# NVIDIA/cuopt

Hardware: AMD Instinct MI355X
Metric: pdlp_iterations_per_sec (higher is better)
Workload: dtype f64; 1 GPU; c3: synthetic random sparse LP S(m=1000000,n=1000000,k=10,seed=2), nnz=10000000, longest row 10, CSR fp64/int32, Stable2 preset, tolerances 0 (fixed iteration budget); rows=1000000, cols=1000000, nnz=10000000, parallelism=single GPU

## Files before the change

### cuopt_amd/capi.py

```python
import ctypes as C
import os

import numpy as np

_HERE = os.path.dirname(os.path.abspath(__file__))
LIB_PATH = os.environ.get("CUOPT_AMD_LIB") or os.path.join(_HERE, "lib", "libcuopt.so")

if not os.path.exists(LIB_PATH):
    raise ImportError(
        "cuopt_amd: %s is missing -- build it with `make -C cuopt_amd/csrc` (or "
        "`python -c 'import __graft_entry__ as g; g.build()'`). There is no CPU fallback." % LIB_PATH)

lib = C.CDLL(LIB_PATH, mode=C.RTLD_GLOBAL)

CUOPT_SUCCESS, CUOPT_INVALID_ARGUMENT, CUOPT_MPS_FILE_ERROR, CUOPT_MPS_PARSE_ERROR = 0, 1, 2, 3
CUOPT_VALIDATION_ERROR, CUOPT_OUT_OF_MEMORY, CUOPT_RUNTIME_ERROR = 4, 5, 6
CUOPT_MINIMIZE, CUOPT_MAXIMIZE = 1, -1
STATUS = {0: "NoTermination", 1: "Optimal", 2: "PrimalInfeasible", 3: "DualInfeasible",
          4: "IterationLimit", 5: "TimeLimit", 6: "NumericalError", 7: "PrimalFeasible",
          8: "FeasibleFound", 9: "ConcurrentLimit"}

c_int, c_double, c_void_p, c_char_p = C.c_int32, C.c_double, C.c_void_p, C.c_char_p
P = C.POINTER


def _f64(a):
    return np.ascontiguousarray(a, dtype=np.float64)


def _i32(a):
    return np.ascontiguousarray(a, dtype=np.int32)


def _ptr(a):
    return None if a is None else a.ctypes.data_as(c_void_p)


class Ctl(C.Structure):
    _fields_ = [("step_size", c_double), ("primal_weight", c_double), ("tau", c_double),
                ("sigma", c_double), ("sum_weights", c_double), ("last_interaction", c_double),
                ("last_movement", c_double), ("last_dx2", c_double), ("last_dy2", c_double),
                ("k", c_int), ("cur", c_int), ("pending_avg", c_int), ("steps_taken", c_int),
                ("attempts", c_int), ("target_steps", c_int), ("error", c_int),
                ("its_since_restart", c_int)]


class StepParams(C.Structure):
    _fields_ = [("reduction_exponent", c_double), ("growth_exponent", c_double),
                ("primal_distance_smoothing", c_double), ("dual_distance_smoothing", c_double)]


class LP(C.Structure):
    _fields_ = [("m", c_int), ("n", c_int), ("offsets", c_void_p), ("indices", c_void_p),
                ("values", c_void_p), ("c", c_void_p), ("lo", c_void_p), ("hi", c_void_p),
                ("lb", c_void_p), ("ub", c_void_p), ("maximize", c_int),
                ("objective_offset", c_double)]


class Hyper(C.Structure):
    _fields_ = [("initial_step_size_scaling", c_double), ("ruiz_iterations", c_int),
                ("do_pock_chambolle", c_int), ("do_ruiz", c_int), ("alpha_pock_chambolle", c_double),
                ("artificial_restart_threshold", c_double),
                ("compute_initial_step_size_before_scaling", c_int),
                ("compute_initial_primal_weight_before_scaling", c_int),
                ("initial_primal_weight_c_scaling", c_double),
                ("initial_primal_weight_b_scaling", c_double), ("major_iteration", c_int),
                ("min_iteration_restart", c_int), ("restart_strategy", c_int),
                ("never_restart_to_average", c_int), ("reduction_exponent", c_double),
                ("growth_exponent", c_double), ("primal_weight_update_smoothing", c_double),
                ("sufficient_reduction_for_restart", c_double),
                ("necessary_reduction_for_restart", c_double), ("primal_importance", c_double),
                ("primal_distance_smoothing", c_double), ("dual_distance_smoothing", c_double),
                ("compute_last_restart_before_new_primal_weight", c_int),
                ("artificial_restart_in_main_loop", c_int), ("rescale_for_restart", c_int),
                ("update_primal_weight_on_initial_solution", c_int),
                ("update_step_size_on_initial_solution", c_int),
                ("handle_some_primal_gradients_on_finite_bounds_as_residuals", c_int),
                ("project_initial_primal", c_int),
                ("algorithm", c_int), ("halpern_power_max_products", c_int),
                ("halpern_step_safety", c_double), ("halpern_power_tolerance", c_double)]


class Halpern(C.Structure):
    _fields_ = [("r", c_double), ("r_first", c_double), ("r2", c_double), ("r2_min", c_double),
                ("k", c_int), ("reserved", c_int)]


class SolverSettings(C.Structure):
    _fields_ = [("absolute_gap_tolerance", c_double), ("relative_gap_tolerance", c_double),
                ("absolute_primal_tolerance", c_double), ("relative_primal_tolerance", c_double),
                ("absolute_dual_tolerance", c_double), ("relative_dual_tolerance", c_double),
                ("iteration_limit", c_int), ("time_limit", c_double),
                ("per_constraint_residual", c_int), ("first_primal_feasible", c_int),
                ("initial_step_size", c_double), ("initial_primal_weight", c_double),
                ("initial_k", c_int), ("use_graph", c_int), ("detect_infeasibility", c_int),
                ("strict_infeasibility", c_int), ("primal_infeasible_tolerance", c_double),
                ("dual_infeasible_tolerance", c_double), ("save_best_primal_so_far", c_int),
                ("log_to_console", c_int), ("log_file", c_char_p), ("unbounded_from_feasible_iterates", c_int),
                ("accept_enabled", c_int), ("accept_tolerance", c_double * 6),
                ("relative_primal_tolerance_factor", c_double), ("relative_dual_tolerance_factor", c_double),
                ("batch_lanes", c_int), ("halpern_resident", c_int), ("halpern_batch", c_int), ("halpern_lockstep", c_int)]


class SolverSettingsWithRays(SolverSettings):
    _fields_ = [("halpern_infeasibility", c_int)]


assert SolverSettingsWithRays.halpern_infeasibility.offset == SolverSettings.halpern_lockstep.offset + C.sizeof(c_int)


class Result(C.Structure):
    _fields_ = [("status", c_int), ("steps_taken", c_int), ("attempted_steps", c_int),
                ("returned_average", c_int), ("num_restarts", c_int), ("num_major_iterations", c_int),
                ("primal_objective", c_double), ("dual_objective", c_double), ("gap", c_double),
                ("relative_gap", c_double), ("l2_primal_residual", c_double),
                ("l2_dual_residual", c_double), ("l2_relative_primal_residual", c_double),
                ("l2_relative_dual_residual", c_double), ("max_primal_ray_infeasibility", c_double),
                ("max_dual_ray_infeasibility", c_double), ("primal_ray_linear_objective", c_double),
                ("dual_ray_linear_objective", c_double), ("initial_step_size", c_double),
                ("initial_primal_weight", c_double), ("step_size", c_double),
                ("primal_weight", c_double), ("norm_b", c_double), ("norm_c", c_double),
                ("setup_seconds", c_double), ("loop_seconds", c_double),
                ("accepted_at_looser_tolerances", c_int), ("gpus", c_int)]

    def as_dict(self):
        d = {k: getattr(self, k) for k, _ in self._fields_}
        d["status_name"] = STATUS.get(self.status, str(self.status))
# ... 141 lines not shown
if hasattr(lib, "pdlpdev_debug_attempts"):
    _proto("pdlpdev_debug_attempts", c_int, c_void_p, c_int, P(Ctl))
_proto("pdlpdev_clear_error", c_int, c_void_p)
_proto("pdlpdev_set_graph_mode", c_int, c_void_p, c_int)
_proto("pdlpdev_prepare_graphs", c_int, c_void_p)
_proto("pdlpdev_flush_average", c_int, c_void_p)
_proto("pdlpdev_make_average", c_int, c_void_p, c_int)
_proto("pdlpdev_eval", c_int, c_void_p, c_int, c_int, c_double, c_double, c_void_p)
_proto("pdlpdev_restart", c_int, c_void_p, c_int, c_int, c_void_p)
_proto("pdlpdev_major_eval", c_int, c_void_p, c_int, c_int, c_double, c_double, c_void_p, c_void_p)
if hasattr(lib, "pdlpdev_loop_stats"):
    _proto("pdlpdev_loop_stats", c_int, c_void_p, c_void_p)
    _proto("pdlpdev_run_period", c_int, c_void_p, c_int, c_void_p, c_void_p, c_void_p, c_void_p, c_void_p)
_proto("pdlpdev_save_best", c_int, c_void_p, c_int)
_proto("pdlpdev_trust_region_bounds", c_int, c_void_p, c_int, c_double, c_double, c_double, c_double, c_double, c_double, c_int, c_void_p)
_proto("pdlpdev_eval_infeasibility", c_int, c_void_p, c_int, c_int, c_void_p)
_proto("pdlpdev_get_solution", c_int, c_void_p, c_int, c_void_p, c_void_p, c_void_p)
_proto("pdlpdev_download", C.c_int64, c_void_p, c_int, c_void_p, C.c_int64)
_proto("pdlpdev_upload", C.c_int64, c_void_p, c_int, c_void_p, C.c_int64)
_proto("pdlpdev_spmv", c_int, c_void_p, c_int, c_void_p, c_void_p)
_proto("pdlpdev_time_kernel", c_int, c_void_p, c_int, c_int, P(c_double))
_proto("pdlpdev_synchronize", c_int, c_void_p)
_proto("pdlpdev_device_bytes", C.c_int64, c_void_p)
_proto("cuoptamd_dual_simplex", c_int, c_void_p, c_double, c_int, c_void_p, c_void_p, c_void_p, c_void_p, c_void_p, c_void_p, c_void_p)
_proto("cuoptamd_dual_simplex_from", c_int, c_void_p, c_void_p, c_void_p, c_double, c_int, c_void_p, c_void_p, c_void_p, c_void_p, c_void_p, c_void_p, c_void_p)
_proto("pdlpdev_shard_dataflow", c_int, c_void_p)
_proto("pdlpdev_shard_transport", c_int, c_void_p)
_proto("pdlpdev_shard_wire_bytes", c_int, c_void_p, c_void_p)
_proto("pdlpdev_dense_info", c_int, c_void_p, c_void_p)
_proto("pdlpdev_layout_info", c_int, c_void_p, c_void_p)
_proto("pdlpdev_comm_abort", c_int, c_void_p)
if hasattr(lib, "pdlpdev_shard_slice"):
    _proto("pdlpdev_shard_slice", c_int, c_void_p, P(c_int), P(c_int))
    _proto("pdlpdev_owner_layout_info", c_int, c_void_p, c_void_p)
_proto("pdlpdev_analyze", c_int, P(c_void_p), c_int, c_int, c_int, c_void_p, c_void_p, c_void_p, c_int)
_proto("pdlpdev_analysis_info", c_int, c_void_p, c_void_p)
_proto("pdlpdev_analysis_maps", c_int, c_void_p, c_void_p, c_void_p)
_proto("pdlpdev_analysis_download", c_int, c_void_p, c_int, c_void_p, c_void_p, c_void_p)
_proto("pdlpdev_create_from_analysis", c_int, P(c_void_p), c_void_p, c_void_p, c_void_p, c_void_p, c_void_p, c_void_p)
_proto("pdlpdev_analysis_destroy", None, c_void_p)
_proto("pdlpdev_debug_sort_pairs", c_int, c_int, C.c_int64, c_void_p, c_void_p, c_int, c_void_p, c_void_p)
_proto("pdlpdev_debug_scan", c_int, c_int, C.c_int64, c_void_p, c_void_p)
_proto("pdlpdev_debug_layout_checksums", c_int, c_void_p, c_void_p)
_proto("cuoptamd_solver_clone", c_int, c_void_p, c_void_p, c_void_p, c_void_p, c_void_p, c_void_p, P(c_void_p))
_proto("cuoptamd_batch_create", c_int, c_void_p, c_int, P(c_void_p))
_proto("cuoptamd_batch_advance", c_int, c_void_p, c_int, c_void_p)
_proto("cuoptamd_batch_destroy", None, c_void_p)
_proto("cuoptamd_batch_reset", c_int, c_void_p, c_void_p, c_void_p, c_void_p, c_void_p)
_proto("cuoptamd_batch_get_solutions", c_int, c_void_p, c_void_p, c_void_p, c_void_p)
_proto("cuoptamd_batch_branch", c_int, c_void_p, c_void_p, c_void_p, c_void_p)
_proto("cuoptamd_batch_solution_views", c_int, c_void_p, c_void_p, c_void_p, c_void_p)
_proto("cuoptamd_batch_device", c_void_p, c_void_p)
_proto("cuoptamd_batch_stats", c_int, c_void_p, c_void_p)
_proto("cuoptamd_batch_solve_last_path", C.c_char_p)
_proto("pdlpdev_small_batch_create", c_int, P(c_void_p), P(c_void_p), c_int)
_proto("pdlpdev_small_batch_destroy", None, c_void_p)
_proto("pdlpdev_create_share_stream", None, c_void_p)
_proto("pdlpdev_debug_ipc_export", c_int, c_int, c_int, c_void_p, P(c_void_p))
_proto("pdlpdev_debug_ipc_store", c_int, c_int, c_void_p, c_int, c_double)
_proto("pdlpdev_debug_ipc_wait", c_int, c_int, c_void_p, c_int, c_double)
_proto("pdlpdev_resident_size", c_int, c_int, c_int, C.c_int64)
if hasattr(lib, "pdlpdev_resident_tier"):
    _proto("pdlpdev_resident_tier", c_int, c_int, c_int, C.c_int64)
_proto("pdlpdev_batch_time_kernels", c_int, c_void_p, c_int, c_void_p)
_proto("pdlpdev_synthetic_lp", c_int, c_int, c_int, c_int, c_int, C.c_uint64, *([c_void_p] * 8))

if hasattr(lib, "pdlpdev_set_halpern"):
    _proto("pdlpdev_create_no_resident", None, c_int)
    _proto("pdlpdev_set_halpern", c_int, c_void_p, c_int)
    _proto("pdlpdev_spectral_norm", c_int, c_void_p, c_double, c_int, P(c_double), P(c_int))
    _proto("pdlpdev_halpern_restart", c_int, c_void_p, c_double, c_void_p, P(Ctl))
    _proto("pdlpdev_get_halpern", c_int, c_void_p, P(Halpern))
if hasattr(lib, "cuoptamd_solver_get_ray"):
    _proto("cuoptamd_solver_get_ray", c_int, c_void_p, c_void_p, c_void_p)
    _proto("pdlpdev_set_halpern_rays", c_int, c_void_p, c_int)
    _proto("pdlpdev_halpern_eval_infeasibility", c_int, c_void_p, c_int, c_void_p)
    _proto("pdlpdev_halpern_get_ray", c_int, c_void_p, c_void_p, c_void_p)
PDLP_SOLVER_MODE_HALPERN1 = 4

BUF = {n: i for i, n in enumerate(
    ["X", "Y", "X_OTHER", "Y_OTHER", "ATY", "ATY_OTHER", "XBAR", "SUM_X", "SUM_Y", "AVG_X", "AVG_Y",
     "DROW", "DCOL", "A_VALUES", "AT_VALUES", "C", "LB", "UB", "LO", "HI", "RC_CURRENT", "RC_AVERAGE",
     "LAST_RESTART_X", "LAST_RESTART_Y", "ATY_U_CURRENT", "ATY_U_AVERAGE", "LAST_RESTART_ATY",
     "AX_U_CURRENT", "AX_U_AVERAGE"])}
KERNEL = {n: i for i, n in enumerate(
    ["PRIMAL", "SPMV_A_DUAL", "SPMV_AT_STEP", "STEP_DECISION", "SPMV_A_PLAIN", "SPMV_AT_PLAIN"])}
EV = {n: i for i, n in enumerate(
    ["CX", "DUAL_SUM", "PRES2", "DRES2", "X2", "Y2", "LINF_PRES_REL", "LINF_DRES_REL"])}
CURRENT, AVERAGE = 0, 1
LAST_RESTART = 2


class CuOptError(RuntimeError):
    def __init__(self, code, msg=""):
        super().__init__("cuopt error %d %s" % (code, msg))
        self.code = code


def device_count():
    return int(lib.pdlpdev_device_count())


def device_info(dev=0):
    name = C.create_string_buffer(256)
    cus, mem = c_int(), C.c_int64()
    rc = lib.pdlpdev_device_info(dev, name, 256, C.byref(cus), C.byref(mem))
    if rc != 0:
        raise CuOptError(rc, lib.pdlpdev_last_error().decode())
    return dict(name=name.value.decode(), compute_units=cus.value, hbm_bytes=mem.value)


class Problem:

    def __init__(self, handle):
        self.handle = handle

    @classmethod
    def read(cls, path):
        h = c_void_p()
        rc = lib.cuOptReadProblem(os.fsencode(path), C.byref(h))
        if rc != CUOPT_SUCCESS:
            raise CuOptError(rc, "cuOptReadProblem(%s)" % path)
        return cls(h)

    @classmethod
    def from_dict(cls, p, ranged=True):
        m, n = int(p["m"]), int(p["n"])
        keep = [_i32(p["offsets"]), _i32(p["indices"]), _f64(p["values"]), _f64(p["c"]),
                _f64(p["lb"]), _f64(p["ub"])]
        vt = p.get("var_types")
        vt = (b"C" * n) if vt is None else bytes(bytearray(np.asarray(vt, dtype=np.uint8)))
        h = c_void_p()
        sense = CUOPT_MAXIMIZE if p.get("maximize", False) else CUOPT_MINIMIZE
        off = float(p.get("objective_offset", 0.0))
        if ranged:
            lo, hi = _f64(p["lo"]), _f64(p["hi"])
            rc = lib.cuOptCreateRangedProblem(m, n, sense, off, _ptr(keep[3]), _ptr(keep[0]),
                                              _ptr(keep[1]), _ptr(keep[2]), _ptr(lo), _ptr(hi),
                                              _ptr(keep[4]), _ptr(keep[5]), vt, C.byref(h))
        else:
            rt = bytes(bytearray(np.asarray(p["row_types"], dtype=np.uint8)))
            rhs = _f64(p["rhs"])
            rc = lib.cuOptCreateProblem(m, n, sense, off, _ptr(keep[3]), _ptr(keep[0]), _ptr(keep[1]),
                                        _ptr(keep[2]), rt, _ptr(rhs), _ptr(keep[4]), _ptr(keep[5]), vt,
                                        C.byref(h))
        if rc != CUOPT_SUCCESS:
            raise CuOptError(rc, "cuOptCreate*Problem")
        return cls(h)

    def _int(self, fn):
        v = c_int()
        rc = fn(self.handle, C.byref(v))
        if rc != 0:
            raise CuOptError(rc)
        return v.value

    @property
    def m(self):
        return self._int(lib.cuOptGetNumConstraints)

    @property
    def n(self):
        return self._int(lib.cuOptGetNumVariables)

    @property
    def nnz(self):
        return self._int(lib.cuOptGetNumNonZeros)
# ... 779 lines not shown
```

### cuopt_amd/csrc/kernels_batch.hip

```cpp
#include <cstring>
#include <hip/hip_runtime.h>

#include "batch_common.hpp"
#include "pdlp_ctx.hpp"

#define LAUNCH_CHECK() HIP_TRY(hipGetLastError())

__global__ void k_step_decision_batch(const pdlpdev_decision_args* __restrict__ args);
__global__ void k_set_target(pdlpdev_ctl* ctl, int target);
__global__ void k_set_error(pdlpdev_ctl* ctl);

namespace {

template <int K>
__global__ void __launch_bounds__(kBT) kb_primal(const BatchLp* __restrict__ lp, int n, double* __restrict__ xK)
{
  __shared__ double tile[kBT][K + 1];
  using WL = WaveLps<K>;
  const int wave = threadIdx.x >> 6, lane = threadIdx.x & 63, sub = WL::sub(wave);
  for (int t0 = blockIdx.x * kBT; t0 < n; t0 += gridDim.x * kBT) {
#pragma unroll
    for (int pass = 0; pass < WL::PASSES; ++pass) {
      const int l       = WL::lp(wave, pass);
      const BatchLp L   = lp[l];
// ... 423 lines not shown
    return batch_halpern_enqueue_tail(K, s, ps, pt, b->lp_dev, b->hl_dev, b->xK, b->yK);
  }
  if (ev) {
    JagView ajv = A.jv, tjv = T.jv;
    int aP = A.P, tP = T.P;
    void* a0[] = {&b->lp_dev, &n, &b->xK};
    void* a1[] = {&aw, &arow0, &c0->A.hot.off, &c0->A.hot.idx, &c0->A.hot.val, &b->lp_dev, &b->xK, &b->yK};
    void* a2[] = {&tw, &trow0, &c0->At.hot.off, &c0->At.hot.idx, &c0->At.hot.val, &b->lp_dev, &b->yK};
    void* j1[] = {&ajv, &aP, &b->lp_dev, &b->xK, &b->yK};
    void* j2[] = {&tjv, &tP, &b->lp_dev, &b->yK};
    void* a3[] = {&b->dargs_dev};
    HIP_TRY(hipExtLaunchKernel((const void*)kb_primal<K>, dim3(pgrid), dim3(kBT), a0, 0, s, ev[0], ev[1], 0));
    if (A.jag)
      HIP_TRY(hipExtLaunchKernel(batch_jag_kernel<K>(A, true), jgrid(A), dim3(A.jv.waves * 64), j1, A.lds, s, ev[2], ev[3], 0));
    else
      HIP_TRY(hipExtLaunchKernel(ap ? (const void*)kb_a_dual<K, 8> : (const void*)kb_a_dual<K, 4>, dim3(aw), dim3(kBT), a1, 0, s, ev[2], ev[3], 0));
    if (T.jag)
      HIP_TRY(hipExtLaunchKernel(batch_jag_kernel<K>(T, false), jgrid(T), dim3(T.jv.waves * 64), j2, T.lds, s, ev[4], ev[5], 0));
    else
      HIP_TRY(hipExtLaunchKernel(tp ? (const void*)kb_at_step<K, 8> : (const void*)kb_at_step<K, 4>, dim3(tw), dim3(kBT), a2, 0, s, ev[4], ev[5], 0));
    HIP_TRY(hipExtLaunchKernel((const void*)k_step_decision_batch, dim3(K), dim3(1024), a3, 0, s, ev[6], ev[7], 0));
    return 0;
  }
  kb_primal<K><<<pgrid, kBT, 0, s>>>(b->lp_dev, n, b->xK);
  if (A.jag && A.jv.waves == 16) kbj_a_dual<K, 16><<<jgrid(A), 1024, A.lds, s>>>(A.jv, A.P, b->lp_dev, b->xK, b->yK);
  else if (A.jag) kbj_a_dual<K, 8><<<jgrid(A), 512, A.lds, s>>>(A.jv, A.P, b->lp_dev, b->xK, b->yK);
  else if (ap) kb_a_dual<K, 8><<<aw, kBT, 0, s>>>(aw, arow0, c0->A.hot.off, c0->A.hot.idx, c0->A.hot.val, b->lp_dev, b->xK, b->yK);
  else kb_a_dual<K, 4><<<aw, kBT, 0, s>>>(aw, arow0, c0->A.hot.off, c0->A.hot.idx, c0->A.hot.val, b->lp_dev, b->xK, b->yK);
  if (T.jag && T.jv.waves == 16) kbj_at_step<K, 16><<<jgrid(T), 1024, T.lds, s>>>(T.jv, T.P, b->lp_dev, b->yK);
  else if (T.jag) kbj_at_step<K, 8><<<jgrid(T), 512, T.lds, s>>>(T.jv, T.P, b->lp_dev, b->yK);
  else if (tp) kb_at_step<K, 8><<<tw, kBT, 0, s>>>(tw, trow0, c0->At.hot.off, c0->At.hot.idx, c0->At.hot.val, b->lp_dev, b->yK);
  else kb_at_step<K, 4><<<tw, kBT, 0, s>>>(tw, trow0, c0->At.hot.off, c0->At.hot.idx, c0->At.hot.val, b->lp_dev, b->yK);
  k_step_decision_batch<<<K, 1024, 0, s>>>(b->dargs_dev);
  LAUNCH_CHECK();
  return 0;
}

static int batch_enqueue(pdlpdev_batch* b, hipEvent_t* ev = nullptr)
{
  return b->K == 16  ? batch_enqueue_attempt<16>(b, ev)
         : b->K == 8 ? batch_enqueue_attempt<8>(b, ev)
         : b->K == 4 ? batch_enqueue_attempt<4>(b, ev)
                     : batch_enqueue_attempt<2>(b, ev);
}

static int batch_graph(pdlpdev_batch* b, int attempts, hipGraphExec_t* out)
{
  auto it = b->graphs.find(attempts);
  if (it != b->graphs.end()) {
    *out = it->second;
    return 0;
  }
  hipGraph_t graph;
  HIP_TRY(hipStreamBeginCapture(b->stream, hipStreamCaptureModeThreadLocal));
  int rc = 0;
  for (int i = 0; i < attempts && rc == 0; ++i) rc = batch_enqueue(b);
  hipError_t e = hipStreamEndCapture(b->stream, &graph);
  if (rc != 0) return rc;
  HIP_TRY(e);
  hipGraphExec_t exec;
  HIP_TRY(hipGraphInstantiate(&exec, graph, nullptr, nullptr, 0));
  HIP_TRY(hipGraphDestroy(graph));
  b->graphs[attempts] = exec;
  *out                = exec;
  return 0;
}

extern "C" {

int pdlpdev_clone_shared(pdlpdev_ctx** out, pdlpdev_ctx* parent)
{
  if (!out || !parent) return fail(-1, "pdlpdev_clone_shared: null argument");
  if (!parent->scaled) return fail(-1, "pdlpdev_clone_shared: the parent has not been scaled yet");
  if (parent->comm || parent->small_resident || parent->dense.on) return fail(-7, "pdlpdev_clone_shared: not for sharded, resident or dense-segment contexts");
  HIP_TRY(hipSetDevice(parent->device));
  HIP_TRY(hipStreamSynchronize(parent->stream));
  pdlpdev_ctx* c = new pdlpdev_ctx(*parent);
  *out           = c;
  c->allocs.clear(), c->graphs.clear(), c->scratch.clear();
  c->shared_with_parent = true;
  c->parent = nullptr;
  c->scal_h = nullptr, c->ctl_h = nullptr;
  c->halpern = false, c->lraty = nullptr, c->hal = nullptr, c->hal_h = nullptr;
  c->clones_alive = 0, c->batches_alive = 0, c->rows_private = false;
  c->bytes = 0, c->slab = nullptr, c->slab_cap = c->slab_used = 0, c->arena = nullptr, c->arena_used = 0, c->first_chunk = nullptr;
  c->bestx = c->besty = c->bestrc = nullptr;
  c->prof_armed = false, c->prof_used = 0, c->rejected_in_a_row = 0;
  for (hipEvent_t& e : c->prof_ev) e = nullptr;
  HIP_TRY(hipHostMalloc((void**)&c->scal_h, kScalars * sizeof(double) + sizeof(pdlpdev_ctl)));
  c->ctl_h = (pdlpdev_ctl*)(c->scal_h + kScalars);
  HIP_TRY(hipMalloc((void**)&c->arena, kArenaChunk));
  HIP_TRY(hipMemsetAsync(c->arena, 0, kArenaChunk, c->stream));
  c->first_chunk = c->arena;
  const int m = c->m, n = c->n;
  {
    const size_t bytes = (24 * ((size_t)n + kSlicePad + 32) + 15 * ((size_t)m + 32)) * sizeof(double);
    if ((int64_t)m + n >= 262144 && hipMalloc((void**)&c->slab, bytes) == hipSuccess) {
      c->allocs.push_back(c->slab);
      c->slab_cap = bytes;
      HIP_TRY(hipMemsetAsync(c->slab, 0, bytes, c->stream));
    } else {
      c->slab = nullptr;
      (void)hipGetLastError();
    }
  }
  auto own_copy = [&](double** p, size_t count) -> int {
    const double* src = *p;
    TRY(dev_alloc(c, p, count));
    HIP_TRY(hipMemcpyAsync(*p, src, count * sizeof(double), hipMemcpyDeviceToDevice, c->stream));
    return 0;
  };
  TRY(own_copy(&c->lb, n)); TRY(own_copy(&c->lb_u, n)); TRY(own_copy(&c->ub, n)); TRY(own_copy(&c->ub_u, n));
  c->rows_aliased = true, c->parent = parent, c->clones_alive = 0;
  parent->clones_alive += 1;
  parent->rows_private = false;
  for (int i = 0; i < 2; ++i) {
    TRY(dev_alloc(c, &c->x[i], (size_t)n + kSlicePad)); TRY(dev_alloc(c, &c->y[i], m));
    TRY(dev_alloc(c, &c->aty[i], (size_t)n + kSlicePad)); TRY(dev_alloc(c, &c->rc[i], n));
  }
  TRY(dev_alloc(c, &c->xbar, (size_t)n + kSlicePad)); TRY(dev_alloc(c, &c->sumx, (size_t)n + kSlicePad)); TRY(dev_alloc(c, &c->sumy, m));
  TRY(dev_alloc(c, &c->avgx, n)); TRY(dev_alloc(c, &c->avgy, m));
  TRY(dev_alloc(c, &c->lrx, n)); TRY(dev_alloc(c, &c->lry, m));
  TRY(dev_alloc(c, &c->tmp_n, n)); TRY(dev_alloc(c, &c->tmp_m, m));
  for (int i = 0; i < 3; ++i) {
    TRY(dev_alloc(c, &c->ax_u[i], m));
    TRY(dev_alloc(c, &c->aty_u[i], n));
  }
  TRY(dev_alloc(c, &c->rc_scratch, n));
  TRY(dev_alloc(c, &c->A.part, (size_t)8 * c->A.max_partials()));
  TRY(dev_alloc(c, &c->At.part, (size_t)8 * c->At.max_partials()));
  TRY(dev_alloc(c, &c->part_g, (size_t)8 * 2048));
  TRY(dev_alloc(c, &c->scal, kScalars));
  TRY(dev_alloc(c, &c->ctl, 1));
  TRY(dev_alloc(c, &c->ar_buf, (size_t)n + kSlicePad));
  HIP_TRY(hipMemcpyAsync(c->ctl, parent->ctl, sizeof(pdlpdev_ctl), hipMemcpyDeviceToDevice, c->stream));
  HIP_TRY(hipStreamSynchronize(c->stream));
  return 0;
}

int pdlpdev_batch_create(pdlpdev_batch** out, pdlpdev_ctx** ctx, int K)
{
  if (!out || !ctx || (K != 2 && K != 4 && K != 8 && K != 16)) return fail(-1, "pdlpdev_batch_create: K must be 2, 4, 8 or 16");
  pdlpdev_ctx* c0 = ctx[0];
  for (int l = 0; l < K; ++l)
    for (int q = 0; q < l; ++q)
      if (ctx[q] == ctx[l]) return fail(-1, "pdlpdev_batch_create: LP %d and LP %d are the same context (two lanes would share one set of iterates)", q, l);
  for (int l = 0; l < K; ++l) {
    pdlpdev_ctx* c = ctx[l];
    if (!c || c->A.hot.off != c0->A.hot.off || c->At.hot.off != c0->At.hot.off || c->A.pan.v.row0 != c0->A.pan.v.row0 || c->A.jag.v.row0 != c0->A.jag.v.row0 ||
        c->At.jag.v.row0 != c0->At.jag.v.row0 || c->A.jag.v.val != c0->A.jag.v.val || c->At.jag.v.val != c0->At.jag.v.val || c->stream != c0->stream)
      return fail(-1, "pdlpdev_batch_create: the contexts do not share one matrix (pdlpdev_clone_shared)");
  }
  int nhalpern = 0;
  for (int l = 0; l < K; ++l) nhalpern += ctx[l]->halpern ? 1 : 0;
  if (nhalpern != 0 && nhalpern != K)
    return fail(-7, "pdlpdev_batch_create: not eligible (the batch mixes %d contexts in reflected Halpern mode with %d in the averaging iteration: a lockstep "
                    "attempt runs one of the two)", nhalpern, K - nhalpern);
  const bool halpern = nhalpern == K;
  for (int l = 0; halpern && l < K; ++l)
    if (!ctx[l]->hal || !ctx[l]->hal_h || !ctx[l]->lraty) return fail(-1, "pdlpdev_batch_create: LP %d is in reflected Halpern mode without its anchor (pdlpdev_set_halpern)", l);
  if ((int64_t)std::max(c0->m, c0->n) * K >= ((int64_t)1 << 32))
    return fail(-7, "pdlpdev_batch_create: not eligible (the interleaved vectors are addressed with 32-bit element offsets: max(m, n) * K < 2^32)");
  pdlpdev_batch::Side side[2];
  HIP_TRY(hipSetDevice(c0->device));
  const pdlpdev_ctx::MatrixSide* const matrix[2] = {&c0->A, &c0->At};
  for (int t = 0; t < 2; ++t) {
// ... 232 lines not shown
```

### cuopt_amd/csrc/kernels_panel.hip

```cpp
#include <hip/hip_runtime.h>

#include "pdlp_kernel_decls.hpp"
#include "pdlp_layouts.hpp"
#include "pdlp_setup.hpp"
#include "spmv_panel.hpp"

template <bool SEG>
__global__ void __launch_bounds__(kPanelThreads)
k_panel_a_dual(PanelView P, const pdlpdev_ctl* __restrict__ ctl, const double* __restrict__ xbar,
               double* __restrict__ y0, double* __restrict__ y1, const double* __restrict__ lo,
               const double* __restrict__ hi, double* __restrict__ sumy, double* __restrict__ part, double* __restrict__ ycopy,
               const p2pdev::Push* __restrict__ push)
{
  if (!loop_active(ctl)) return;
  DualEpilogue e = DualEpilogue::make(ctl, y0, y1, lo, hi, sumy, ycopy, push);
  panel_block<SEG>(P, xbar, e, part);
  if (push) p2pdev::count_exchange(push);
}

template <bool SEG>
__global__ void __launch_bounds__(kPanelThreads)
k_panel_at_step(PanelView P, const pdlpdev_ctl* __restrict__ ctl, const double* __restrict__ y0,
                const double* __restrict__ y1, const double* __restrict__ x0,
                const double* __restrict__ x1, double* __restrict__ aty0, double* __restrict__ aty1,
                double* __restrict__ part)
{
  if (!loop_active(ctl)) return;
  StepEpilogue e = StepEpilogue::make(ctl, x0, x1, aty0, aty1);
  panel_block<SEG>(P, ctl->cur ? y0 : y1 , e, part);
}

template <bool SEG>
__global__ void __launch_bounds__(kPanelThreads)
k_panel_a_halpern(PanelView P, const pdlpdev_ctl* __restrict__ ctl, const double* __restrict__ xbar,
                  double* __restrict__ y0, double* __restrict__ y1, const double* __restrict__ lo,
                  const double* __restrict__ hi, HalpernArgs h, double* __restrict__ part)
{
  if (!loop_active(ctl)) return;
  HalpernDualEpilogue e = HalpernDualEpilogue::make(ctl, y0, y1, lo, hi, h);
  panel_block<SEG>(P, xbar, e, part);
}

template <bool SEG>
__global__ void __launch_bounds__(kPanelThreads)
k_panel_at_halpern(PanelView P, const pdlpdev_ctl* __restrict__ ctl, double* __restrict__ x0, double* __restrict__ x1,
                   double* __restrict__ aty0, double* __restrict__ aty1, HalpernArgs h, double* __restrict__ part)
{
  if (!loop_active(ctl)) return;
  HalpernStepEpilogue e = HalpernStepEpilogue::make(ctl, x0, x1, aty0, aty1, h);
  panel_block<SEG>(P, h.ty , e, part);
}

template <bool SEG>
__global__ void __launch_bounds__(kPanelThreads)
k_panel_at_cur(PanelView P, const pdlpdev_ctl* __restrict__ ctl, const double* __restrict__ y0,
               const double* __restrict__ y1, double* __restrict__ aty0, double* __restrict__ aty1,
               double* __restrict__ out_override, int use_next)
{
  const int cur = ctl->cur ^ (use_next ? 1 : 0);
  StoreEpilogue e = StoreEpilogue::iterate(cur, aty0, aty1, out_override);
  panel_block<SEG>(P, cur ? y1 : y0, e, nullptr);
}

template <bool SEG>
__global__ void __launch_bounds__(kPanelThreads)
k_panel_plain(PanelView P, const double* __restrict__ vec, double* __restrict__ out)
{
  StoreEpilogue e{out};
  panel_block<SEG>(P, vec, e, nullptr);
}

template <bool SEG>
__global__ void __launch_bounds__(kPanelThreads)
k_panel_eval_primal(PanelView P, const pdlpdev_ctl* __restrict__ ctl, int which,
                    const double* __restrict__ x0, const double* __restrict__ x1,
                    const double* __restrict__ avgx, const double* __restrict__ y0,
                    const double* __restrict__ y1, const double* __restrict__ avgy,
                    const double* __restrict__ dr, const double* __restrict__ lo_u,
                    const double* __restrict__ hi_u, double eps_rel, double* __restrict__ linf_rows,
                    double* __restrict__ ax_out, double* __restrict__ part)
{
  if (period_guard_skips(ctl, which)) return;
  const int cur = ctl->cur;
  const double* xv = evaluated(cur, which, x0, x1, avgx);
  const double* yv = evaluated(cur, which, y0, y1, avgy);
  EvalPrimalEpilogue e{yv, dr, lo_u, hi_u, eps_rel, linf_rows, ax_out};
  panel_block<SEG>(P, xv, e, part);
}

template <bool SEG>
__global__ void __launch_bounds__(kPanelThreads)
k_panel_eval_dual(PanelView P, const pdlpdev_ctl* __restrict__ ctl, int which,
                  const double* __restrict__ x0, const double* __restrict__ x1,
                  const double* __restrict__ avgx, const double* __restrict__ y0,
                  const double* __restrict__ y1, const double* __restrict__ avgy, EvalDualCore core,
                  double* __restrict__ part)
{
  if (period_guard_skips(ctl, which)) return;
  const int cur = ctl->cur;
// ... 331 lines not shown
```

### cuopt_amd/csrc/pdlp_create.hip

```cpp
#include "pdlp_ctx.hpp"
#include "pdlp_layouts.hpp"
#include "pdlp_setup.hpp"

__global__ void k_fill(int64_t n, double* __restrict__ d, double v);
int sync_panel_values(pdlpdev_ctx* c);
int resident_tier(int m, int n, int64_t nnz);

static thread_local int g_create_sharded = 0;
static thread_local int g_create_no_resident = 0;
static thread_local int g_create_batch_lanes = 0;

static int create_impl(pdlpdev_ctx** out, int device, int32_t m, int32_t n, const int32_t* a_offsets,
                       const int32_t* a_indices, const double* a_values, const int32_t* at_offsets,
                       const int32_t* at_indices, const double* at_values,
                       void (*transpose_ready)(void*), void* user, const double* c, const double* lo,
                       const double* hi, const double* lb, const double* ub, pdlpdev_analysis* an);

extern "C" {

const char* pdlpdev_last_error(void) { return g_err.c_str(); }
void pdlpdev_create_hint(int sharded) { g_create_sharded = sharded; }
void pdlpdev_create_no_resident(int no_resident) { g_create_no_resident = no_resident; }
void pdlpdev_create_batch_lanes(int lanes) { g_create_batch_lanes = lanes; }
static thread_local pdlpdev_ctx* g_create_stream_donor = nullptr;
// ... 446 lines not shown
      if (!hT_off.empty()) T.off = hT_off.data(), T.idx = hT_idx.data();
      rbt = build_row_blocks(n, T.off);
      wlap("row blocks");
      if (walk) at_rc = layout_walk(ctx, P, T);
    };
    struct Join {
      std::thread t;
      ~Join() { if (t.joinable()) t.join(); }
    } worker;
    if (at_thread) worker.t = std::thread(at_side, true);
    {
      LayoutSide A;
      init_side(A, &ctx->A, 0);
      A.off = A_off, A.idx = A_idx, A.d_off = ctx->A.hot.off, A.d_idx = ctx->A.hot.idx, A.d_val = ctx->A.hot.val, A.lap = lap;
      A.first_seg = DH.on ? &DH.first_seg : nullptr;
      TRY(layout_walk(ctx, P, A));
      TRY(upload_side(ctx, P, A));
      if (ctx->A.pan.on && DH.on) TRY(own_segments(ctx, DH, A.ph));
      lap("upload layouts A");
    }
    if (at_thread) worker.t.join();
    else at_side(false);
    lap("wait for the A^T side");
    if ((int64_t)at_offsets[n] != ctx->nnz) return fail(-1, "pdlpdev_create: A and A^T disagree on nnz");
    if (!an) {
      TRY(upload_i32(ctx, &ctx->At.full.off, at_offsets, (size_t)n + 1));
      TRY(upload_i32(ctx, &ctx->At.full.idx, at_indices, nnz, 8));
      TRY(upload_f64(ctx, &ctx->At.full.val, at_values, nnz, 8));
    }
    ctx->At.nlong = (int)lat.size();
    if (ctx->At.nlong) TRY(upload_i32(ctx, &ctx->At.longs, lat.data(), lat.size()));
    const bool hot_t = !hT_off.empty();
    ctx->At.hot = ctx->At.full;
    ctx->At.hot_nnz = (int64_t)T.off[n];
    if (hot_t) {
      TRY(upload_i32(ctx, &ctx->At.hot.off, T.off, (size_t)n + 1));
      TRY(upload_i32(ctx, &ctx->At.hot.idx, T.idx, (size_t)ctx->At.hot_nnz, 8));
      TRY(dev_alloc(ctx, &ctx->At.hot.val, (size_t)ctx->At.hot_nnz + 8));
      TRY(upload_i32(ctx, &ctx->dense.s_perm_at, hT_perm.data(), hT_perm.size()));
    }
    if (DH.on) TRY(dev_alloc(ctx, &ctx->At.dense_add, (size_t)n));
    ctx->At.nb = (int)rbt.size() / 2 - 1;
    TRY(upload_i32(ctx, &ctx->At.rb, rbt.data(), rbt.size()));
    lap("upload A^T");
    T.d_off = ctx->At.hot.off, T.d_idx = ctx->At.hot.idx, T.d_val = ctx->At.hot.val;
    TRY(at_thread ? at_rc : layout_walk(ctx, P, T));
    TRY(upload_side(ctx, P, T));
    if (ctx->At.pan.on && DH.on) TRY(column_segments(ctx, DH, T.ph));
    lap("upload layouts A^T");
    HIP_TRY(hipStreamSynchronize(ctx->stream));
  }
  {
    const char* small_env = getenv("CUOPT_AMD_SMALL");
    const int tier        = resident_tier(m, n, ctx->nnz);
    ctx->eval_reuse_aty   = cuopt_amd::tune_int("eval_reuse_aty", 1) != 0;
    ctx->small_resident   = tier >= 0 && !(small_env && atoi(small_env) == 0) && !ctx->A.dense_add && !ctx->At.dense_add && !g_create_no_resident;
    g_create_no_resident  = 0;
    if (small_env && atoi(small_env) != 0 && tier < 0)
      return fail(-1, "CUOPT_AMD_SMALL=1: the LP does not fit the resident kernel (m, n <= 2048, nnz <= 4096 ...)");
  }
  ctx->slab_cap += slab_rest;
  for (pdlpdev_ctx::MatrixSide* s : {&ctx->A, &ctx->At}) {
    s->pan.v.dense_add = s->jag.v.dense_add = s->pb.v.dense_add = s->dense_add;
    if (s->pan.v.dn_own_seg || s->pan.v.dn_pan_ptr) s->pan.v.dense_add = nullptr;
    TRY(dev_alloc(ctx, &s->part, (size_t)8 * s->max_partials()));
  }
  TRY(dev_alloc(ctx, &ctx->part_g, (size_t)8 * 2048));
  TRY(dev_alloc(ctx, &ctx->scal, kScalars));
  TRY(dev_alloc(ctx, &ctx->ctl, 1));
  TRY(dev_alloc(ctx, &ctx->ar_buf, (size_t)n + kSlicePad));
  lap("partial buffers");
  k_fill<<<grid_for(m), kBlock, 0, ctx->stream>>>(m, ctx->dr, 1.0);
  k_fill<<<grid_for(n), kBlock, 0, ctx->stream>>>(n, ctx->dc, 1.0);
  HIP_TRY(hipGetLastError());
  lap("fill D");
  TRY(sync_panel_values(ctx));
  lap("panel values (permute)");
  if (P.mode == LayoutPolicy::kTimed) {
    TRY(pick_layout(ctx, &ctx->A, ctx->tmp_n, ctx->tmp_m));
    lap("layout autotune A");
    TRY(pick_layout(ctx, &ctx->At, ctx->tmp_m, ctx->tmp_n));
    lap("layout autotune");
  }
  HIP_TRY(hipStreamSynchronize(ctx->stream));
  scratch_free(ctx);
  return 0;
}

extern "C" {

void pdlpdev_destroy(pdlpdev_ctx* ctx)
{
  if (!ctx) return;
  (void)hipSetDevice(ctx->device);
  if (ctx->stream) (void)hipStreamSynchronize(ctx->stream);
  scratch_free(ctx);
  for (auto& kv : ctx->graphs) (void)hipGraphExecDestroy(kv.second);
  if (ctx->shared_with_parent && ctx->parent) ctx->parent->clones_alive -= 1;
  if (ctx->batches_alive > 0)
    fprintf(stderr, "[cuopt_amd] pdlpdev_destroy: %d batch(es) still hold this context -- destroy the batch before its members\n", ctx->batches_alive);
  if (ctx->clones_alive > 0)
    fprintf(stderr, "[cuopt_amd] pdlpdev_destroy: %d clone(s) of this context are still alive -- they alias its matrices and must be destroyed first\n", ctx->clones_alive);
  for (void* mapped : ctx->p2p.opened) (void)hipIpcCloseMemHandle(mapped);
  if (ctx->p2p.base) (void)hipFree(ctx->p2p.base);
  if (ctx->comm && !ctx->soft) comm_cache::release(ctx->comm_key);
  for (void* p : ctx->allocs) (void)hipFree(p);
  if (ctx->hal_h) (void)hipHostFree(ctx->hal_h);
  const bool whole = ctx->stream && ctx->scal_h && ctx->first_chunk && !ctx->shared_with_parent && !ctx->stream_borrowed;
  if (!(whole && give_recycled(Recycled{ctx->device, ctx->stream, ctx->scal_h, ctx->first_chunk}))) {
    if (ctx->first_chunk) (void)hipFree(ctx->first_chunk);
    if (ctx->scal_h) (void)hipHostFree(ctx->scal_h);
    if (ctx->stream && !ctx->shared_with_parent && !ctx->stream_borrowed) (void)hipStreamDestroy(ctx->stream);
  }
  delete ctx;
}

}
```

### cuopt_amd/csrc/pdlp_ctx.hpp

```cpp
#pragma once
#include <hip/hip_runtime.h>
#include <hip/hip_ext.h>

#include <tuple>
#include <utility>

#include <dlfcn.h>
#include <unistd.h>
#include <mutex>
#include <math.h>
#include <stdarg.h>
#include <stdio.h>
#include <string.h>

#include <algorithm>
#include <chrono>
#include <map>
#include <memory>
#include <string>
#include <vector>

#include "host_parallel.hpp"
#include "pdlp_kernels.hpp"
#include "pdlp_epilogues.hpp"
// ... 276 lines not shown
    int32_t* rb = nullptr;
    int nb = 0;
    int32_t* longs = nullptr;
    int nlong = 0;
    Panels pan;
    Jag jag;
    Pb pb;
    double* part = nullptr;
    double* dense_add = nullptr;
    enum Layout { kStream = 0, kPanel = 1, kJag = 3, kPb = 4 };
    Layout layout() const { return pb.on ? kPb : jag.on ? kJag : pan.on ? kPanel : kStream; }
    int partials() const
    {
      switch (layout()) {
        case kPb: return pb.v.B;
        case kJag: return jag.v.nblk + jag.v.nlong;
        case kPanel: return pan.v.W;
        default: return nb;
      }
    }
    int max_partials() const { return std::max({nb, pb.on ? pb.v.B : 0, pan.on ? pan.v.W : 0, jag.on ? jag.v.nblk + jag.v.nlong : 0, 1}); }
    void info(int32_t out[3]) const
    {
      out[0] = layout();
      switch (layout()) {
        case kPb: out[1] = pb.v.B, out[2] = (int)(100.0 * (pb.pad - 1.0) + 0.5); break;
        case kJag: out[1] = jag.v.nblk, out[2] = (int)(100.0 * jag.saving + 0.5); break;
        case kPanel: out[1] = pan.v.W, out[2] = pan.v.S; break;
        default: out[1] = nb, out[2] = 1;
      }
    }
    bool fuses_dense() const { return pan.on && (pan.v.dn_own_seg != nullptr || pan.v.dn_pan_ptr != nullptr); }
  };
  MatrixSide A, At;
  struct Dense {
    bool on = false;
    int nrows = 0, nseg = 0, ntiles = 0;
    int64_t nent = 0;
    int32_t *row = nullptr, *row_seg = nullptr;
    int32_t *seg_row = nullptr, *seg_c0 = nullptr, *seg_len = nullptr, *seg_ptr = nullptr;
    int32_t *ch_seg = nullptr, *ch_k0 = nullptr, *row_ch = nullptr;
    double* ch_part = nullptr;
    int nchunks = 0;
    int32_t *tile_ptr = nullptr, *tile_seg = nullptr, *tile_id = nullptr;
    int32_t *perm = nullptr, *s_perm_a = nullptr, *s_perm_at = nullptr;
    double* val = nullptr;
    int32_t* tile_slot = nullptr;
  } dense;
  double *c = nullptr, *lb = nullptr, *ub = nullptr, *lo = nullptr, *hi = nullptr;
  struct UniformBounds {
    int lb_same = 0, ub_same = 0;
    double lb = 0.0, ub = 0.0;
  } ubd;
  void note_uniform_bounds(const double* lb_host, const double* ub_host)
  {
    auto same = [&](const double* v, int* flag, double* value) {
      if (!v) return;
      *flag = 0;
      if (n <= 0) return;
      const double v0 = v[0];
      if (!(v0 == 0.0 || std::isinf(v0))) return;
      constexpr int kParts = 16;
      bool differs[kParts] = {false};
      cuopt_amd::parallel_tasks(kParts, [&](int t) {
        const int32_t a = (int32_t)((int64_t)n * t / kParts), b = (int32_t)((int64_t)n * (t + 1) / kParts);
        for (int32_t j = a; j < b; ++j)
          if (v[j] != v0) {
            differs[t] = true;
            return;
          }
      }, (int64_t)n * 4);
      for (bool d : differs)
        if (d) return;
      *flag = 1, *value = v0;
    };
    same(lb_host, &ubd.lb_same, &ubd.lb);
    same(ub_host, &ubd.ub_same, &ubd.ub);
  }
  double *c_u = nullptr, *lb_u = nullptr, *ub_u = nullptr, *lo_u = nullptr, *hi_u = nullptr;
  double *dr = nullptr, *dc = nullptr;
  bool scaled = false;
  double *x[2] = {nullptr, nullptr}, *y[2] = {nullptr, nullptr}, *aty[2] = {nullptr, nullptr};
  double *xbar = nullptr, *sumx = nullptr, *sumy = nullptr, *avgx = nullptr, *avgy = nullptr;
  double *lrx = nullptr, *lry = nullptr, *rc[2] = {nullptr, nullptr};
  double *tmp_n = nullptr, *tmp_m = nullptr;
  double *ax_u[3] = {nullptr, nullptr, nullptr}, *aty_u[3] = {nullptr, nullptr, nullptr};
  double* rc_scratch = nullptr;
  double *bestx = nullptr, *besty = nullptr, *bestrc = nullptr;
  double *part_g = nullptr;
  double *scal = nullptr;
  double *scal_h = nullptr;
  pdlpdev_ctl *ctl = nullptr, *ctl_h = nullptr;
  pdlpdev_step_params sp = {0.3, 0.6, 0.5, 0.5};
  bool halpern = false;
  double* lraty = nullptr;
  pdlpdev_halpern *hal = nullptr, *hal_h = nullptr;
  bool halpern_rays = false;
  rccl::comm_t comm = nullptr;
  softcomm::Comm* soft = nullptr;
  std::string comm_key;
  int rank = 0, world = 1;
  double* ar_buf = nullptr;
  bool rsag = false;
  int slice = 0;
  double* rs_buf = nullptr;
  double* rs_scal = nullptr;
  bool owner = false;
  int ypad = 0;
  double* ygather = nullptr;
  MatrixSide Oc;
  struct Halo {
    bool on = false;
    std::vector<int32_t> recv_off[2], recv_cnt[2], send_off[2], send_cnt[2];
    int64_t bytes = 0, bytes_allgather = 0;
  } halo;
  struct P2P {
    bool on = false;
    char* base = nullptr;
    size_t bytes = 0;
    size_t off_x = 0, off_y = 0, off_s = 0, off_f = 0;
    p2pdev::Peers peers{};
    std::vector<void*> opened;
    unsigned long long* epoch = nullptr;
    int* fault = nullptr;
    p2pdev::Push* push_dev = nullptr;
    p2pdev::Push push_host[p2pdev::kKinds];
  } p2p;
  bool prof_armed = false;
  static constexpr int kProfPairs = 8;
  hipEvent_t prof_ev[2 * kProfPairs] = {};
  int prof_used = 0;
  int rejected_in_a_row = 0;
  bool aty_valid = false, ctl_h_current = false;
  int eval_reuse_aty = 1;
  int spare_attempts = 0;
  int64_t stat_eval_reused = 0, stat_eval_product = 0, stat_loop_syncs = 0, stat_empty_attempts = 0;
  int use_graph = 1;
  int batch_lanes = 0;
  bool comm_warm = false;
  bool graph_comm_failed = false;
  char* slab = nullptr;
  size_t slab_cap = 0, slab_used = 0;
  char* arena = nullptr;
  char* first_chunk = nullptr;
  bool stream_borrowed = false;
  size_t arena_used = 0;
  bool small_resident = false;
  bool shared_with_parent = false;
  pdlpdev_ctx* parent = nullptr;
  bool rows_aliased = false;
  int clones_alive = 0;
  bool rows_private = false;
  int batches_alive = 0;
  std::map<int, hipGraphExec_t> graphs;
  std::vector<void*> allocs;
  int64_t bytes = 0;
  struct Scratch {
    void* p;
    size_t bytes;
    bool busy;
  };
  std::vector<Scratch> scratch;
};
inline int scratch_take(pdlpdev_ctx* c, void** p, size_t bytes)
{
  bytes = std::max<size_t>(bytes, 256);
// ... 137 lines not shown
```

### cuopt_amd/csrc/pdlp_device.hip

```cpp
#include "pdlp_ctx.hpp"
#include "pdlp_layouts.hpp"
#include "pdlp_setup.hpp"
#include "halpern_decision.hpp"


__global__ void __launch_bounds__(kBlock) k_fill(int64_t n, double* __restrict__ d, double v)
{
  for (int64_t i = blockIdx.x * (int64_t)kBlock + threadIdx.x; i < n; i += (int64_t)gridDim.x * kBlock)
    d[i] = v;
}
__global__ void __launch_bounds__(kBlock) k_scale_vectors(int n, int m, double* __restrict__ c,
                                                          double* __restrict__ lb,
                                                          double* __restrict__ ub,
                                                          const double* __restrict__ dc,
                                                          double* __restrict__ lo,
                                                          double* __restrict__ hi,
                                                          const double* __restrict__ dr)
{
  const int tot = n > m ? n : m;
  for (int i = blockIdx.x * kBlock + threadIdx.x; i < tot; i += gridDim.x * kBlock) {
    if (i < n) {
      c[i]  = c[i] * dc[i];
      lb[i] = lb[i] / dc[i];
      ub[i] = ub[i] / dc[i];
// ... 1 lines not shown
    if (i < m) {
      lo[i] = lo[i] * dr[i];
      hi[i] = hi[i] * dr[i];
    }
  }
}
__global__ void __launch_bounds__(kBlock) k_scale_bounds(int n, int m, double* lb, double* ub,
                                                         const double* __restrict__ dc, double* lo, double* hi,
                                                         const double* __restrict__ dr)
{
  const int tot = n > m ? n : m;
  for (int i = blockIdx.x * kBlock + threadIdx.x; i < tot; i += gridDim.x * kBlock) {
    if (i < n) {
      if (lb) lb[i] = lb[i] / dc[i];
      if (ub) ub[i] = ub[i] / dc[i];
    }
    if (i < m) {
      if (lo) lo[i] = lo[i] * dr[i];
      if (hi) hi[i] = hi[i] * dr[i];
    }
  }
}
__global__ void __launch_bounds__(kBlock) k_div_inplace(int n, double* __restrict__ v,
                                                        const double* __restrict__ d)
{
  for (int i = blockIdx.x * kBlock + threadIdx.x; i < n; i += gridDim.x * kBlock) v[i] = v[i] / d[i];
}
__global__ void __launch_bounds__(kBlock) k_div_to(int n, double* __restrict__ out, const double* __restrict__ v,
                                                   const double* __restrict__ d)
{
  for (int i = blockIdx.x * kBlock + threadIdx.x; i < n; i += gridDim.x * kBlock) out[i] = v[i] / d[i];
}
__global__ void __launch_bounds__(kBlock) k_clamp(int n, double* __restrict__ x,
                                                  const double* __restrict__ lb,
                                                  const double* __restrict__ ub)
{
  for (int i = blockIdx.x * kBlock + threadIdx.x; i < n; i += gridDim.x * kBlock)
    x[i] = dmin(dmax(x[i], lb[i]), ub[i]);
}

template <int MODE>
__global__ void __launch_bounds__(kBlock) k_reduce(int64_t n, const double* __restrict__ a,
                                                   const double* __restrict__ b,
                                                   double* __restrict__ part)
{
  __shared__ double red[8];
  double acc[1] = {0.0};
  for (int64_t i = blockIdx.x * (int64_t)kBlock + threadIdx.x; i < n; i += (int64_t)gridDim.x * kBlock) {
    if (MODE == 0) {
      const double v = fabs(a[i]);
      acc[0] = v > acc[0] ? v : acc[0];
    } else if (MODE == 1) {
      acc[0] += a[i] * a[i];
    } else if (MODE == 2) {
      const double v = combine_bounds(a[i], b[i]);
      acc[0] += v * v;
    } else {
      const double v = a[i] - b[i];
      acc[0] += v * v;
    }
  }
  if (MODE == 0)
    block_reduce<MaxOp, 1>(acc, red);
  else
    block_reduce<SumOp, 1>(acc, red);
  if (threadIdx.x == 0) part[blockIdx.x] = acc[0];
}
__global__ void __launch_bounds__(kBlock) k_dot(int64_t n, const double* __restrict__ a, const double* __restrict__ b,
                                                double* __restrict__ part)
{
  __shared__ double red[8];
  double acc[1] = {0.0};
  for (int64_t i = blockIdx.x * (int64_t)kBlock + threadIdx.x; i < n; i += (int64_t)gridDim.x * kBlock) acc[0] += a[i] * b[i];
  block_reduce<SumOp, 1>(acc, red);
  if (threadIdx.x == 0) part[blockIdx.x] = acc[0];
}
__global__ void __launch_bounds__(kBlock) k_finalize(const double* __restrict__ part, int nb, int nq,
                                                     unsigned op_mask, double* __restrict__ out)
{
  __shared__ double red[8];
  finalize_rows(part, nb, nq, op_mask, out, red);
}

__global__ void __launch_bounds__(kBlock)
k_primal(int n, const pdlpdev_ctl* __restrict__ ctl, double* __restrict__ x0, double* __restrict__ x1,
         const double* __restrict__ aty0, const double* __restrict__ aty1,
         const double* __restrict__ c, const double* __restrict__ lb, const double* __restrict__ ub,
         double* __restrict__ xbar, double* __restrict__ sumx, const p2pdev::Push* __restrict__ push, pdlpdev_ctx::UniformBounds ubd)
{
  if (!loop_active(ctl)) return;
  const int cur       = ctl->cur;
  const double tau    = ctl->tau;
  const double weight = ctl->step_size;
  const bool pend     = ctl->pending_avg != 0;
  const double* __restrict__ x   = cur ? x1 : x0;
  double* __restrict__ xn        = cur ? x0 : x1;
  const double* __restrict__ aty = cur ? aty1 : aty0;
  for (int j = blockIdx.x * kBlock + threadIdx.x; j < n; j += gridDim.x * kBlock) {
    const double xj       = x[j];
    const double gradient = c[j] - aty[j];
    double next           = xj - (tau * gradient);
    next                  = dmax(dmin(next, ubd.ub_same ? ubd.ub : ub[j]), ubd.lb_same ? ubd.lb : lb[j]);
    xn[j]                 = next;
    const double xb       = next - xj + next;
    xbar[j]               = xb;
    if (push)
      for (int q = 0; q < push->world; ++q)
        if (push->wants(q, j)) p2pdev::put(push->slot(q) + j, xb);
    if (pend) sumx[j] = sumx[j] + weight * xj;
  }
  if (push) p2pdev::count_exchange(push);
}



__global__ void __launch_bounds__(kBlock)
k_step_stats(int n, int nbg, const pdlpdev_ctl* __restrict__ ctl, const double* __restrict__ reduced,
             const double* __restrict__ x0, const double* __restrict__ x1, double* __restrict__ aty0,
             double* __restrict__ aty1, double* __restrict__ part)
{
  __shared__ double red[12];
  if (!loop_active(ctl)) return;
  const int cur = ctl->cur;
  const double* __restrict__ x   = cur ? x1 : x0;
  const double* __restrict__ xn  = cur ? x0 : x1;
  const double* __restrict__ aty = cur ? aty1 : aty0;
  double* __restrict__ atyn      = cur ? aty0 : aty1;
  double acc[2] = {0.0, 0.0};
  for (int j = blockIdx.x * kBlock + threadIdx.x; j < n; j += gridDim.x * kBlock) {
    const double v  = reduced[j];
    atyn[j]         = v;
    const double dx = xn[j] - x[j];
    const double t  = v - aty[j];
    acc[0] += t * dx;
    acc[1] += dx * dx;
  }
  block_reduce<SumOp, 2>(acc, red);
  if (threadIdx.x == 0) {
    part[blockIdx.x]       = acc[0];
    part[nbg + blockIdx.x] = acc[1];
  }
}

constexpr int kDecisionThreads = 1024;
static_assert(kDecisionThreads == kHalpernDecisionThreads, "k_halpern_decision runs halpern_decision_workgroup");
__device__ __forceinline__ void step_decision_workgroup(pdlpdev_ctl* __restrict__ ctl, const double* __restrict__ part_dy, int nb_dy,
                                                        const double* __restrict__ part_t, int nb_t, const double* __restrict__ dy2_reduced,
                                                        const pdlpdev_step_params& sp)
{
  __shared__ double red[3 * 16];
  __shared__ double pw[2];
  pdlpdev_ctl lc = *ctl;
  if (!(lc.error == 0 && lc.steps_taken < lc.target_steps)) return;
  const int t = threadIdx.x;
  if (t >= kDecisionThreads - 2) {
    const double knext = (double)(lc.k + 1) + 1.0;
    pw[t - (kDecisionThreads - 2)] = pow(knext, t == kDecisionThreads - 2 ? -sp.reduction_exponent : -sp.growth_exponent);
  }
  double acc[3] = {0.0, 0.0, 0.0};
  if (dy2_reduced == nullptr) {
#pragma unroll 4
    for (int i = t; i < nb_dy; i += kDecisionThreads) acc[0] += part_dy[i];
  }
#pragma unroll 4
  for (int i = t; i < nb_t; i += kDecisionThreads) {
    acc[1] += part_t[i];
    acc[2] += part_t[nb_t + i];
  }
  block_sum_fast<3, kDecisionThreads / 64>(acc, red);
  if (t != 0) return;
  apply_step_decision(&lc, dy2_reduced ? dy2_reduced[0] : acc[0], acc[1], acc[2], sp, pw);
  *ctl = lc;
}
__global__ void __launch_bounds__(kDecisionThreads)
k_step_decision(pdlpdev_ctl* __restrict__ ctl, const double* __restrict__ part_dy, int nb_dy,
                const double* __restrict__ part_t, int nb_t, const double* __restrict__ dy2_reduced,
                pdlpdev_step_params sp)
{
  step_decision_workgroup(ctl, part_dy, nb_dy, part_t, nb_t, dy2_reduced, sp);
}
__global__ void __launch_bounds__(kDecisionThreads)
k_step_decision_batch(const pdlpdev_decision_args* __restrict__ args)
{
  const pdlpdev_decision_args a = args[blockIdx.x];
  step_decision_workgroup(a.ctl, a.part_dy, a.nb_dy, a.part_t, a.nb_t, nullptr, a.sp);
}

__global__ void __launch_bounds__(kDecisionThreads)
k_halpern_decision(pdlpdev_ctl* __restrict__ ctl, pdlpdev_halpern* __restrict__ hal, const double* __restrict__ part_dy, int nb_dy,
                   const double* __restrict__ part_t, int nb_t)
{
  halpern_decision_workgroup(ctl, hal, part_dy, nb_dy, part_t, nb_t);
}
__global__ void k_halpern_clear(pdlpdev_halpern* hal)
{
  hal->r = hal->r_first = hal->r2 = 0.0;
  hal->r2_min = __builtin_huge_val();
  hal->k = 0, hal->reserved = 0;
}
__global__ void k_halpern_restart_ctl(pdlpdev_ctl* ctl, pdlpdev_halpern* hal, double* dist2, double theta)
{
  const double dx = sqrt(dist2[0]), dy = sqrt(dist2[1]);
  dist2[0] = dx, dist2[1] = dy;
  if (theta >= 0.0 && dx > 1.0e-10 && dy > 1.0e-10) {
    const double w     = exp(theta * log(dy / dx) + (1.0 - theta) * log(ctl->primal_weight));
    ctl->primal_weight = w;
    ctl->tau           = ctl->step_size / w;
    ctl->sigma         = ctl->step_size * w;
  }
  ctl->its_since_restart = 0;
  hal->k                 = 0;
}
__global__ void __launch_bounds__(kBlock)
k_copy_current(int n, const pdlpdev_ctl* __restrict__ ctl, const double* __restrict__ v0, const double* __restrict__ v1, double* __restrict__ out)
{
  const double* __restrict__ v = ctl->cur ? v1 : v0;
  for (int i = blockIdx.x * kBlock + threadIdx.x; i < n; i += gridDim.x * kBlock) out[i] = v[i];
}
__global__ void __launch_bounds__(kBlock) k_div_by_scalar(int n, double* __restrict__ out, const double* __restrict__ v, double d)
{
  for (int i = blockIdx.x * kBlock + threadIdx.x; i < n; i += gridDim.x * kBlock) out[i] = v[i] / d;
}

__global__ void __launch_bounds__(kBlock)
k_step_decision_p2p(pdlpdev_ctl* __restrict__ ctl, const double* __restrict__ part_dy, int nb_dy, const double* __restrict__ part_t, int nb_t,
                    const double* __restrict__ landed, const unsigned long long* __restrict__ flags, int world,
                    const unsigned long long* __restrict__ epoch, int* __restrict__ fault, pdlpdev_step_params sp, const p2pdev::Push* __restrict__ push)
{
  if (!loop_active(ctl)) return;
  {
    __shared__ double red[3 * 8];
    double acc[3] = {0.0, 0.0, 0.0};
    for (int i = threadIdx.x; i < nb_dy; i += kBlock) acc[0] += part_dy[i];
    for (int i = threadIdx.x; i < nb_t; i += kBlock) {
      acc[1] += part_t[i];
      acc[2] += part_t[nb_t + i];
    }
    block_reduce<SumOp, 3>(acc, red);
    if (threadIdx.x == 0) {
      for (int q = 0; q < push->world; ++q) {
        double* d = push->slot(q);
        p2pdev::put(d, acc[0]), p2pdev::put(d + 1, acc[1]), p2pdev::put(d + 2, acc[2]);
      }
      asm volatile("s_waitcnt vmcnt(0)" ::: "memory");
      push->epoch[push->kind] = push->epoch[push->kind] + 1;
      p2pdev::raise(push);
    }
    __syncthreads();
  }
  if (!p2pdev::wait_flags(flags, world, 2, epoch)) {
    if (threadIdx.x == 0) *fault = 1, ctl->error = 1;
    return;
  }
  if (threadIdx.x != 0) return;
  double sum[3] = {0.0, 0.0, 0.0};
  for (int q = 0; q < world; ++q)
    for (int k = 0; k < 3; ++k) sum[k] += __hip_atomic_load(landed + 4 * q + k, __ATOMIC_RELAXED, __HIP_MEMORY_SCOPE_SYSTEM);
  pdlpdev_ctl lc = *ctl;
  apply_step_decision(&lc, sum[0], sum[1], sum[2], sp);
  *ctl = lc;
}

// ... 423 lines not shown
    k_div_inplace<<<grid_for(ctx->n), kBlock, 0, ctx->stream>>>(ctx->n, ctx->x[cur], ctx->dc);
  }
  if (y) {
    HIP_TRY(hipMemcpyAsync(ctx->y[cur], y, (size_t)ctx->m * sizeof(double), hipMemcpyHostToDevice, ctx->stream));
    k_div_inplace<<<grid_for(ctx->m), kBlock, 0, ctx->stream>>>(ctx->m, ctx->y[cur], ctx->dr);
  }
  LAUNCH_CHECK();
  HIP_TRY(hipStreamSynchronize(ctx->stream));
  return 0;
}
}
extern "C" {
int pdlpdev_initial_solution_stats(pdlpdev_ctx* ctx, double out[5], const double* x0_unscaled, const double* y0_unscaled)
{
  HIP_TRY(hipSetDevice(ctx->device));
  if ((x0_unscaled == nullptr) != (y0_unscaled == nullptr)) return fail(-1, "initial_solution_stats: both unscaled vectors or none");
  hipStream_t s = ctx->stream;
  const int n = ctx->n, m = ctx->m;
  TRY(fetch_ctl(ctx, nullptr));
  const int cur = ctx->ctl_h->cur;
  const double *xv = ctx->x[cur], *yv = ctx->y[cur], *atyv = ctx->aty[cur];
  if (x0_unscaled) {
    const int nxt = 1 - cur;
    HIP_TRY(hipMemcpyAsync(ctx->x[nxt], x0_unscaled, (size_t)n * sizeof(double), hipMemcpyHostToDevice, s));
    HIP_TRY(hipMemcpyAsync(ctx->y[nxt], y0_unscaled, (size_t)m * sizeof(double), hipMemcpyHostToDevice, s));
    double* prod = ctx->comm ? ctx->ar_buf : ctx->aty[nxt];
    launch_plain(ctx, 1, ctx->y[nxt], prod);
    LAUNCH_CHECK();
    if (ctx->comm) TRY(allreduce(ctx, prod, (size_t)n, rccl::kSum));
    xv = ctx->x[nxt], yv = ctx->y[nxt], atyv = prod;
  } else {
    TRY(pdlpdev_compute_aty(ctx));
  }
  const int g = std::min(grid_for(n), kGenericBlocks);
  k_dot<<<g, kBlock, 0, s>>>(n, xv, atyv, ctx->part_g);
  k_finalize<<<1, kBlock, 0, s>>>(ctx->part_g, g, 1, 0u, ctx->scal + 48);
  TRY(reduce_vec(ctx, 1, n, xv, nullptr, 49));
  TRY(reduce_vec(ctx, 1, m, yv, nullptr, 50));
  TRY(reduce_vec(ctx, 0, n, xv, nullptr, 51));
  TRY(reduce_vec(ctx, 0, m, yv, nullptr, 52));
  LAUNCH_CHECK();
  if (ctx->comm) {
    TRY(allreduce(ctx, ctx->scal + 50, 1, rccl::kSum));
    TRY(allreduce(ctx, ctx->scal + 52, 1, rccl::kMax));
  }
  HIP_TRY(hipMemcpyAsync(ctx->scal_h + 48, ctx->scal + 48, 5 * sizeof(double), hipMemcpyDeviceToHost, s));
  HIP_TRY(hipStreamSynchronize(s));
  for (int i = 0; i < 5; ++i) out[i] = ctx->scal_h[48 + i];
  return 0;
}

int pdlpdev_project_primal(pdlpdev_ctx* ctx)
{
  HIP_TRY(hipSetDevice(ctx->device));
  TRY(fetch_ctl(ctx, nullptr));
  const int cur = ctx->ctl_h->cur;
  k_clamp<<<grid_for(ctx->n), kBlock, 0, ctx->stream>>>(ctx->n, ctx->x[cur], ctx->lb, ctx->ub);
  k_clamp<<<grid_for(ctx->n), kBlock, 0, ctx->stream>>>(ctx->n, ctx->avgx, ctx->lb, ctx->ub);
  LAUNCH_CHECK();
  return 0;
}

}
extern "C" {
int pdlpdev_compute_aty(pdlpdev_ctx* ctx)
{
  HIP_TRY(hipSetDevice(ctx->device));
  hipStream_t s = ctx->stream;
  if (!ctx->comm) {
    launch_at_cur(ctx, nullptr, 0);
    LAUNCH_CHECK();
  } else {
    launch_at_cur(ctx, ctx->ar_buf, 0);
    LAUNCH_CHECK();
    TRY(allreduce(ctx, ctx->ar_buf, (size_t)ctx->n, rccl::kSum));
    TRY(fetch_ctl(ctx, nullptr));
    HIP_TRY(hipMemcpyAsync(ctx->aty[ctx->ctl_h->cur], ctx->ar_buf, (size_t)ctx->n * sizeof(double), hipMemcpyDeviceToDevice, s));
  }
  return 0;
}


static inline HalpernArgs halpern_args(const pdlpdev_ctx* ctx) { return HalpernArgs{ctx->hal, ctx->avgx, ctx->avgy, ctx->lrx, ctx->lry, ctx->lraty}; }
static void launch_a_dual(pdlpdev_ctx* ctx, double* ycopy = nullptr, const p2pdev::Push* push = nullptr)
{
  const Gathered g = Gathered::fixed(ctx->xbar, true);
  const auto pre  = std::make_tuple(ctx->ctl);
  const auto vecs = std::make_tuple(ctx->xbar);
  if (ctx->halpern) (void)launch_product(ctx, ctx->A, products::a_halpern, g, pre, vecs, std::make_tuple(ctx->y[0], ctx->y[1], ctx->lo, ctx->hi, halpern_args(ctx), ctx->A.part));
  else (void)launch_product(ctx, ctx->A, products::a_dual, g, pre, vecs, std::make_tuple(ctx->y[0], ctx->y[1], ctx->lo, ctx->hi, ctx->sumy, ctx->A.part, ycopy, push));
}
static void launch_at_step(pdlpdev_ctx* ctx)
{
  const auto pre = std::make_tuple(ctx->ctl);
  if (ctx->halpern)
    (void)launch_product(ctx, ctx->At, products::at_halpern, Gathered::fixed(ctx->avgy, true), pre, std::make_tuple(),
                         std::make_tuple(ctx->x[0], ctx->x[1], ctx->aty[0], ctx->aty[1], halpern_args(ctx), ctx->At.part));
  else
    (void)launch_product(ctx, ctx->At, products::at_step, Gathered::trial(ctx->y[0], ctx->y[1], true), pre, std::make_tuple(ctx->y[0], ctx->y[1]),
                         std::make_tuple(ctx->x[0], ctx->x[1], ctx->aty[0], ctx->aty[1], ctx->At.part));
}
void launch_at_cur(pdlpdev_ctx* ctx, double* out_override, int use_next)
{
  (void)launch_product(ctx, ctx->At, products::at_cur, use_next ? Gathered::trial(ctx->y[0], ctx->y[1]) : Gathered::current(ctx->y[0], ctx->y[1]), std::make_tuple(ctx->ctl),
                       std::make_tuple(ctx->y[0], ctx->y[1]), std::make_tuple(ctx->aty[0], ctx->aty[1], out_override, use_next));
}
void launch_plain(pdlpdev_ctx* ctx, int transpose, const double* vec, double* out)
{
  (void)launch_product(ctx, transpose ? ctx->At : ctx->A, products::plain, Gathered::fixed(vec), std::make_tuple(), std::make_tuple(vec), std::make_tuple(out));
}
static void launch_decision(pdlpdev_ctx* ctx)
{
  if (ctx->halpern) return launch_k(ctx, k_halpern_decision, 1, kDecisionThreads, 0, ctx->ctl, ctx->hal, ctx->A.part, ctx->A.partials(), ctx->At.part, ctx->At.partials());
  launch_k(ctx, k_step_decision, 1, kDecisionThreads, 0, ctx->ctl, ctx->A.part, ctx->A.partials(), ctx->At.part, ctx->At.partials(), nullptr, ctx->sp);
}

static void launch_oc_step(pdlpdev_ctx* ctx)
{
  const size_t cs = (size_t)ctx->rank * ctx->slice;
  double *x0 = ctx->x[0] + cs, *x1 = ctx->x[1] + cs, *t0 = ctx->aty[0] + cs, *t1 = ctx->aty[1] + cs;
  const double* yg = ctx->ygather;
  (void)launch_product(ctx, ctx->Oc, products::at_step, Gathered::trial(yg, yg, true), std::make_tuple(ctx->ctl), std::make_tuple(yg, yg),
                       std::make_tuple(x0, x1, t0, t1, ctx->Oc.part));
}

static int enqueue_attempt(pdlpdev_ctx* ctx)
{
  const int n = ctx->n;
  if (ctx->halpern && ctx->comm) return fail(-7, "reflected Halpern mode: not available behind a communicator");
  if (ctx->owner) {
    if (!ctx->Oc.hot.off) return fail(-1, "owner-computes dataflow: pdlpdev_owner_setup was not called");
    const size_t cs = (size_t)ctx->rank * ctx->slice;
    const int len   = (int)std::max<int64_t>(0, std::min<int64_t>(ctx->slice, (int64_t)n - (int64_t)cs));
    launch_k(ctx, k_primal, grid_for(len), kBlock, 0, len, ctx->ctl, ctx->x[0] + cs, ctx->x[1] + cs, ctx->aty[0] + cs, ctx->aty[1] + cs,
             ctx->c + cs, ctx->lb + cs, ctx->ub + cs, ctx->xbar + cs, ctx->sumx + cs, ctx->p2p.on ? ctx->p2p.push_dev : (const p2pdev::Push*)nullptr, ctx->ubd);
    LAUNCH_CHECK();
    if (ctx->p2p.on) {
      pdlpdev_ctx::P2P& P = ctx->p2p;
      const int W = ctx->world;
      const unsigned long long* flags = reinterpret_cast<const unsigned long long*>(P.base + P.off_f);
      auto pull = [&](int kind, double* dst, size_t land_off, int per_rank) {
        const int count = W * per_rank, remote = count - per_rank;
        const int g     = std::max(1, std::min((remote + 4095) / 4096, 1024));
        launch_k(ctx, p2pdev::k_pull, g, 256, 0, ctx->ctl, dst, reinterpret_cast<const double*>(P.base + land_off), count, ctx->rank * per_rank, per_rank,
                 flags, W, kind, P.epoch, P.fault, P.push_dev + kind);
      };
      auto pull_ranges = [&](int kind, double* dst, size_t land_off) {
        p2pdev::PullRanges R{};
        int most = 0;
        for (int q = 0; q < W; ++q) R.off[q] = ctx->halo.recv_off[kind][q], R.cnt[q] = ctx->halo.recv_cnt[kind][q], most = std::max(most, R.cnt[q]);
        launch_k(ctx, p2pdev::k_pull_ranges, std::max(1, std::min((most + 255) / 256, 64)), 256, 0, ctx->ctl, dst, reinterpret_cast<const double*>(P.base + land_off), R, flags, W,
                 kind, P.epoch, P.fault, P.push_dev + kind);
      };
      if (ctx->halo.on) pull_ranges(0, ctx->xbar, P.off_x);
      else pull(0, ctx->xbar, P.off_x, ctx->slice);
      launch_a_dual(ctx, ctx->ygather + (size_t)ctx->rank * ctx->ypad, P.push_dev + 1);
      if (ctx->halo.on) pull_ranges(1, ctx->ygather, P.off_y);
      else pull(1, ctx->ygather, P.off_y, ctx->ypad);
      launch_oc_step(ctx);
      launch_k(ctx, k_step_decision_p2p, 1, kBlock, 0, ctx->ctl, ctx->A.part, ctx->A.partials(), ctx->Oc.part, ctx->Oc.partials(),
               reinterpret_cast<const double*>(P.base + P.off_s), flags, W, P.epoch, P.fault, ctx->sp, P.push_dev + 2);
      LAUNCH_CHECK();
      return 0;
    }
    if (ctx->halo.on) TRY(halo_exchange(ctx, 0, ctx->xbar));
    else TRY(all_gather(ctx, ctx->xbar, (size_t)ctx->slice));
    launch_a_dual(ctx, ctx->ygather + (size_t)ctx->rank * ctx->ypad);
    LAUNCH_CHECK();
    if (ctx->halo.on) TRY(halo_exchange(ctx, 1, ctx->ygather));
    else TRY(all_gather(ctx, ctx->ygather, (size_t)ctx->ypad));
    launch_oc_step(ctx);
    launch_k(ctx, k_pack_step_sums, 1, kBlock, 0, ctx->A.part, ctx->A.partials(), ctx->Oc.part, ctx->Oc.partials(), ctx->rs_scal);
    LAUNCH_CHECK();
    TRY(allreduce(ctx, ctx->rs_scal, 3, rccl::kSum));
    launch_k(ctx, k_step_decision, 1, kDecisionThreads, 0, ctx->ctl, nullptr, 0, ctx->rs_scal + 1, 1, ctx->rs_scal, ctx->sp);
    LAUNCH_CHECK();
    return 0;
  }
  if (ctx->rsag) {
    const size_t cs = (size_t)ctx->rank * ctx->slice;
    const int len   = (int)std::max<int64_t>(0, std::min<int64_t>(ctx->slice, (int64_t)n - (int64_t)cs));
    launch_k(ctx, k_primal, grid_for(len), kBlock, 0, len, ctx->ctl, ctx->x[0] + cs, ctx->x[1] + cs, ctx->aty[0] + cs, ctx->aty[1] + cs,
             ctx->c + cs, ctx->lb + cs, ctx->ub + cs, ctx->xbar + cs, ctx->sumx + cs, (const p2pdev::Push*)nullptr, ctx->ubd);
    LAUNCH_CHECK();
    TRY(all_gather(ctx, ctx->xbar, (size_t)ctx->slice));
    launch_a_dual(ctx);
    launch_at_cur(ctx, ctx->ar_buf, 1);
    LAUNCH_CHECK();
    TRY(reduce_scatter(ctx, ctx->ar_buf, ctx->rs_buf, (size_t)ctx->slice));
    const int g = std::min(grid_for(len), kGenericBlocks);
    launch_k(ctx, k_step_stats, g, kBlock, 0, len, g, ctx->ctl, ctx->rs_buf, ctx->x[0] + cs, ctx->x[1] + cs, ctx->aty[0] + cs, ctx->aty[1] + cs, ctx->part_g);
    launch_k(ctx, k_pack_step_sums, 1, kBlock, 0, ctx->A.part, ctx->A.partials(), ctx->part_g, g, ctx->rs_scal);
    LAUNCH_CHECK();
    TRY(allreduce(ctx, ctx->rs_scal, 3, rccl::kSum));
    launch_k(ctx, k_step_decision, 1, kDecisionThreads, 0, ctx->ctl, nullptr, 0, ctx->rs_scal + 1, 1, ctx->rs_scal, ctx->sp);
    LAUNCH_CHECK();
    return 0;
  }
  launch_k(ctx, k_primal, grid_for(n), kBlock, 0, n, ctx->ctl, ctx->x[0], ctx->x[1], ctx->aty[0], ctx->aty[1], ctx->c, ctx->lb, ctx->ub, ctx->xbar, ctx->sumx, (const p2pdev::Push*)nullptr, ctx->ubd);
  launch_a_dual(ctx);
  if (!ctx->comm) {
    launch_at_step(ctx);
    launch_decision(ctx);
  } else {
    launch_at_cur(ctx, ctx->ar_buf, 1);
    launch_k(ctx, k_sum_partials_to, 1, kBlock, 0, ctx->A.part, ctx->A.partials(), ctx->ar_buf + n);
    LAUNCH_CHECK();
    TRY(allreduce(ctx, ctx->ar_buf, (size_t)n + 1, rccl::kSum));
    const int g = std::min(grid_for(n), kGenericBlocks);
    launch_k(ctx, k_step_stats, g, kBlock, 0, n, g, ctx->ctl, ctx->ar_buf, ctx->x[0], ctx->x[1], ctx->aty[0], ctx->aty[1], ctx->part_g);
    launch_k(ctx, k_step_decision, 1, kDecisionThreads, 0, ctx->ctl, nullptr, 0, ctx->part_g, g, ctx->ar_buf + n, ctx->sp);
  }
  LAUNCH_CHECK();
  return 0;
}

static int get_graph(pdlpdev_ctx* ctx, int attempts, hipGraphExec_t* out)
{
  auto it = ctx->graphs.find(attempts);
  if (it != ctx->graphs.end()) {
    *out = it->second;
    return 0;
  }
  hipGraph_t graph;
  HIP_TRY(hipStreamBeginCapture(ctx->stream, hipStreamCaptureModeThreadLocal));
  int rc = 0;
  for (int i = 0; i < attempts && rc == 0; ++i) rc = enqueue_attempt(ctx);
  hipError_t e = hipStreamEndCapture(ctx->stream, &graph);
  if (rc != 0) return rc;
  HIP_TRY(e);
  hipGraphExec_t exec;
  HIP_TRY(hipGraphInstantiate(&exec, graph, nullptr, nullptr, 0));
  HIP_TRY(hipGraphDestroy(graph));
  ctx->graphs[attempts] = exec;
  *out                  = exec;
  return 0;
}

static int enqueue_attempts(pdlpdev_ctx* ctx, int remaining)
{
  const bool rccl_graphs = ctx->comm && !ctx->p2p.on && !ctx->soft && !ctx->graph_comm_failed;
  bool replayed = false;
  if (rccl_graphs && ctx->use_graph && !ctx->comm_warm) {
    TRY(enqueue_attempt(ctx));
    ctx->comm_warm = true;
    remaining -= 1;
  }
  if (ctx->use_graph && (!ctx->comm || ctx->p2p.on || rccl_graphs)) {
    replayed = true;
    while (remaining > 0) {
      int chunk = 1;
      while (chunk * 2 <= remaining && chunk < 64) chunk *= 2;
      hipGraphExec_t g;
      const int grc = get_graph(ctx, chunk, &g);
      if (grc != 0 && rccl_graphs) {
        ctx->graph_comm_failed = true;
        (void)hipGetLastError();
        replayed = false;
        break;
      }
      TRY(grc);
      HIP_TRY(hipGraphLaunch(g, ctx->stream));
      remaining -= chunk;
    }
  }
  if (!replayed) {
    for (int i = 0; i < remaining; ++i) TRY(enqueue_attempt(ctx));
  }
  return 0;
}

static int after_round(pdlpdev_ctx* ctx, int before, int attempts_before, int enqueued, int counted )
{
  const pdlpdev_ctl& c = *ctx->ctl_h;
  const int made       = c.attempts - attempts_before;
  if (!ctx->comm) ctx->stat_empty_attempts += enqueued - made;
  if (c.steps_taken > before && c.error == 0 && !ctx->comm) ctx->aty_valid = true;
  if (c.error != 0) ctx->aty_valid = false;
  if (ctx->p2p.on && c.error != 0) {
    int fault = 0;
    HIP_TRY(hipMemcpy(&fault, ctx->p2p.fault, sizeof(int), hipMemcpyDeviceToHost));
    if (fault) return fail(-6, "direct peer transport: rank %d waited 5 s for another rank's data (a peer failed or is stuck)", ctx->rank);
// ... 207 lines not shown
int pdlpdev_set_graph_mode(pdlpdev_ctx* ctx, int use_graph)
{
  ctx->use_graph = use_graph;
  return 0;
}

int pdlpdev_get_solution(pdlpdev_ctx* ctx, int which, double* x, double* y, double* rc)
{
  HIP_TRY(hipSetDevice(ctx->device));
  TRY(fetch_ctl(ctx, nullptr));
  const int cur = ctx->ctl_h->cur;
  hipStream_t s = ctx->stream;
  if (which == PDLPDEV_BEST) {
    if (!ctx->bestx) return fail(-1, "pdlpdev_get_solution(BEST): nothing was saved");
    if (x) {
      k_unscale<<<grid_for(ctx->n), kBlock, 0, s>>>(ctx->n, ctx->bestx, ctx->dc, ctx->tmp_n);
      HIP_TRY(hipMemcpyAsync(x, ctx->tmp_n, (size_t)ctx->n * sizeof(double), hipMemcpyDeviceToHost, s));
    }
    if (y) {
      k_unscale<<<grid_for(ctx->m), kBlock, 0, s>>>(ctx->m, ctx->besty, ctx->dr, ctx->tmp_m);
      HIP_TRY(hipMemcpyAsync(y, ctx->tmp_m, (size_t)ctx->m * sizeof(double), hipMemcpyDeviceToHost, s));
    }
    if (rc) HIP_TRY(hipMemcpyAsync(rc, ctx->bestrc, (size_t)ctx->n * sizeof(double), hipMemcpyDeviceToHost, s));
    LAUNCH_CHECK();
    HIP_TRY(hipStreamSynchronize(s));
    return 0;
  }
  if (x) {
    k_unscale<<<grid_for(ctx->n), kBlock, 0, s>>>(ctx->n, which == PDLPDEV_AVERAGE ? ctx->avgx : ctx->x[cur], ctx->dc, ctx->tmp_n);
    HIP_TRY(hipMemcpyAsync(x, ctx->tmp_n, (size_t)ctx->n * sizeof(double), hipMemcpyDeviceToHost, s));
  }
  if (y) {
    k_unscale<<<grid_for(ctx->m), kBlock, 0, s>>>(ctx->m, which == PDLPDEV_AVERAGE ? ctx->avgy : ctx->y[cur], ctx->dr, ctx->tmp_m);
    HIP_TRY(hipMemcpyAsync(y, ctx->tmp_m, (size_t)ctx->m * sizeof(double), hipMemcpyDeviceToHost, s));
  }
  if (rc)
    HIP_TRY(hipMemcpyAsync(rc, ctx->rc[which == PDLPDEV_AVERAGE ? 1 : 0], (size_t)ctx->n * sizeof(double), hipMemcpyDeviceToHost, s));
  LAUNCH_CHECK();
  HIP_TRY(hipStreamSynchronize(s));
  return 0;
}

static int64_t locate_buffer(pdlpdev_ctx* ctx, int id, double** ptr)
{
  if (hipSetDevice(ctx->device) != hipSuccess) return -2;
  if (fetch_ctl(ctx, nullptr) != 0) return -2;
  const int cur = ctx->ctl_h->cur;
  double* src   = nullptr;
  int64_t count = 0;
  const int64_t n = ctx->n, m = ctx->m, nnz = ctx->nnz;
  switch (id) {
    case PDLPDEV_BUF_X: src = ctx->x[cur], count = n; break;
    case PDLPDEV_BUF_Y: src = ctx->y[cur], count = m; break;
    case PDLPDEV_BUF_X_OTHER: src = ctx->x[cur ^ 1], count = n; break;
    case PDLPDEV_BUF_Y_OTHER: src = ctx->y[cur ^ 1], count = m; break;
    case PDLPDEV_BUF_ATY: src = ctx->aty[cur], count = n; break;
    case PDLPDEV_BUF_ATY_OTHER: src = ctx->aty[cur ^ 1], count = n; break;
    case PDLPDEV_BUF_XBAR: src = ctx->xbar, count = n; break;
    case PDLPDEV_BUF_SUM_X: src = ctx->sumx, count = n; break;
    case PDLPDEV_BUF_SUM_Y: src = ctx->sumy, count = m; break;
    case PDLPDEV_BUF_AVG_X: src = ctx->avgx, count = n; break;
    case PDLPDEV_BUF_AVG_Y: src = ctx->avgy, count = m; break;
    case PDLPDEV_BUF_DROW: src = ctx->dr, count = m; break;
    case PDLPDEV_BUF_DCOL: src = ctx->dc, count = n; break;
    case PDLPDEV_BUF_A_VALUES: src = ctx->A.full.val, count = nnz; break;
    case PDLPDEV_BUF_AT_VALUES: src = ctx->At.full.val, count = nnz; break;
    case PDLPDEV_BUF_C: src = ctx->c, count = n; break;
    case PDLPDEV_BUF_LB: src = ctx->lb, count = n; break;
    case PDLPDEV_BUF_UB: src = ctx->ub, count = n; break;
    case PDLPDEV_BUF_LO: src = ctx->lo, count = m; break;
    case PDLPDEV_BUF_HI: src = ctx->hi, count = m; break;
    case PDLPDEV_BUF_RC_CURRENT: src = ctx->rc[0], count = n; break;
    case PDLPDEV_BUF_RC_AVERAGE: src = ctx->rc[1], count = n; break;
    case PDLPDEV_BUF_LAST_RESTART_X: src = ctx->lrx, count = n; break;
    case PDLPDEV_BUF_LAST_RESTART_Y: src = ctx->lry, count = m; break;
    case PDLPDEV_BUF_ATY_U_CURRENT: src = ctx->aty_u[PDLPDEV_CURRENT], count = n; break;
    case PDLPDEV_BUF_ATY_U_AVERAGE: src = ctx->aty_u[PDLPDEV_AVERAGE], count = n; break;
    case PDLPDEV_BUF_LAST_RESTART_ATY:
      if (!ctx->lraty) { fail(-1, "buffer %d exists in Halpern mode only", id); return -1; }
      src = ctx->lraty, count = n;
      break;
    case PDLPDEV_BUF_AX_U_CURRENT: src = ctx->ax_u[PDLPDEV_CURRENT], count = m; break;
    case PDLPDEV_BUF_AX_U_AVERAGE: src = ctx->ax_u[PDLPDEV_AVERAGE], count = m; break;
    default: fail(-1, "unknown buffer %d", id); return -1;
  }
  *ptr = src;
  return count;
}

int64_t pdlpdev_download(pdlpdev_ctx* ctx, int id, void* host, int64_t max_elements)
{
  double* src   = nullptr;
  int64_t count = locate_buffer(ctx, id, &src);
  if (count < 0) return count;
  count = std::min(count, max_elements);
  if (count > 0) {
    if (hipMemcpyAsync(host, src, (size_t)count * sizeof(double), hipMemcpyDeviceToHost, ctx->stream) != hipSuccess) return -2;
    if (hipStreamSynchronize(ctx->stream) != hipSuccess) return -2;
  }
  return count;
}

int64_t pdlpdev_upload(pdlpdev_ctx* ctx, int id, const void* host, int64_t elements)
{
  double* dst   = nullptr;
  int64_t count = locate_buffer(ctx, id, &dst);
  if (count < 0) return count;
  if (id == PDLPDEV_BUF_A_VALUES || id == PDLPDEV_BUF_AT_VALUES) {
    fail(-1, "matrix values cannot be overwritten");
    return -1;
  }
  count = std::min(count, elements);
  ctx->aty_valid = false;
  if ((id == PDLPDEV_BUF_LB && ctx->ubd.lb_same) || (id == PDLPDEV_BUF_UB && ctx->ubd.ub_same)) {
    if (id == PDLPDEV_BUF_LB) ctx->ubd.lb_same = 0;
    else ctx->ubd.ub_same = 0;
    for (auto& kv : ctx->graphs) (void)hipGraphExecDestroy(kv.second);
    ctx->graphs.clear();
  }
  if (count > 0) {
    if (hipMemcpyAsync(dst, host, (size_t)count * sizeof(double), hipMemcpyHostToDevice, ctx->stream) != hipSuccess) return -2;
    if (hipStreamSynchronize(ctx->stream) != hipSuccess) return -2;
  }
  return count;
}

int pdlpdev_set_loop_state(pdlpdev_ctx* ctx, double sum_weights, int32_t its_since_restart, int32_t k)
{
  HIP_TRY(hipSetDevice(ctx->device));
  loop_state_touched(ctx);
  k_set_loop_state<<<1, 1, 0, ctx->stream>>>(ctx->ctl, sum_weights, its_since_restart, k);
  LAUNCH_CHECK();
  return 0;
}

static void drop_graphs(pdlpdev_ctx* ctx)
{
  for (auto& kv : ctx->graphs) (void)hipGraphExecDestroy(kv.second);
  ctx->graphs.clear();
}
int pdlpdev_set_halpern(pdlpdev_ctx* ctx, int on)
{
  HIP_TRY(hipSetDevice(ctx->device));
  if ((on != 0) == ctx->halpern) return 0;
  if (on) {
    if (ctx->comm) return fail(-7, "reflected Halpern mode: not available for a sharded solver");
    if (!ctx->scaled) return fail(-1, "pdlpdev_set_halpern: call after pdlpdev_scale_problem");
    if (!ctx->lraty) TRY(dev_alloc(ctx, &ctx->lraty, (size_t)ctx->n));
    if (!ctx->hal) TRY(dev_alloc(ctx, &ctx->hal, 1));
    if (!ctx->hal_h) HIP_TRY(hipHostMalloc((void**)&ctx->hal_h, sizeof(pdlpdev_halpern)));
    k_halpern_clear<<<1, 1, 0, ctx->stream>>>(ctx->hal);
    LAUNCH_CHECK();
    *ctx->hal_h        = pdlpdev_halpern{};
    ctx->hal_h->r2_min = HUGE_VAL;
  }
  ctx->halpern = on != 0;
  loop_state_touched(ctx);
  drop_graphs(ctx);
  return 0;
}
int pdlpdev_get_halpern(pdlpdev_ctx* ctx, pdlpdev_halpern* out)
{
  if (!ctx->halpern) return fail(-1, "pdlpdev_get_halpern: the context is not in Halpern mode");
  *out = *ctx->hal_h;
  return 0;
}
int pdlpdev_spectral_norm(pdlpdev_ctx* ctx, double rel_tol, int32_t max_products, double* sigma_max, int32_t* products)
{
  HIP_TRY(hipSetDevice(ctx->device));
  if (ctx->comm) return fail(-7, "pdlpdev_spectral_norm: single GPU only");
  hipStream_t s = ctx->stream;
  const int n   = ctx->n;
  double* v = ctx->tmp_n;
  k_fill<<<grid_for(n), kBlock, 0, s>>>(n, v, 1.0 / sqrt((double)n));
  double est = 0.0;
  int done   = 0;
  while (done < max_products) {
    launch_plain(ctx, 0, v, ctx->tmp_m);
    launch_plain(ctx, 1, ctx->tmp_m, ctx->xbar);
    TRY(reduce_vec(ctx, 1, n, ctx->xbar, nullptr, 0));
    TRY(fetch_scalars(ctx, 1));
    done += 1;
    const double s2 = sqrt(ctx->scal_h[0]);
    if (!(s2 > 0.0)) {
      est = 0.0;
      break;
    }
    k_div_by_scalar<<<grid_for(n), kBlock, 0, s>>>(n, v, ctx->xbar, s2);
    LAUNCH_CHECK();
    const bool settled = fabs(s2 - est) <= rel_tol * s2;
    est                = s2;
    if (settled) break;
  }
  HIP_TRY(hipMemsetAsync(ctx->xbar, 0, (size_t)n * sizeof(double), s));
  if (sigma_max) *sigma_max = sqrt(est);
  if (products) *products = done;
  return 0;
}
int pdlpdev_halpern_restart(pdlpdev_ctx* ctx, double theta, double dist[2], pdlpdev_ctl* ctl)
{
  HIP_TRY(hipSetDevice(ctx->device));
  if (!ctx->halpern) return fail(-1, "pdlpdev_halpern_restart: the context is not in Halpern mode");
  hipStream_t s = ctx->stream;
  const int g   = std::min(grid_for(std::max(ctx->n, ctx->m)), kGenericBlocks);
  launch_restart_current(ctx, g);
  k_finalize<<<1, kBlock, 0, s>>>(ctx->part_g, g, 2, 0u, ctx->scal);
  k_copy_current<<<grid_for(ctx->n), kBlock, 0, s>>>(ctx->n, ctx->ctl, ctx->aty[0], ctx->aty[1], ctx->lraty);
  k_halpern_restart_ctl<<<1, 1, 0, s>>>(ctx->ctl, ctx->hal, ctx->scal, theta);
  LAUNCH_CHECK();
  HIP_TRY(hipMemcpyAsync(ctx->scal_h, ctx->scal, 2 * sizeof(double), hipMemcpyDeviceToHost, s));
  TRY(fetch_ctl(ctx, ctl));
  ctx->stat_loop_syncs += 1;
  if (dist) dist[0] = ctx->scal_h[0], dist[1] = ctx->scal_h[1];
  return 0;
}

int pdlpdev_spmv(pdlpdev_ctx* ctx, int transpose, const double* x, double* y)
{
  HIP_TRY(hipSetDevice(ctx->device));
  hipStream_t s  = ctx->stream;
  const int rows = transpose ? ctx->n : ctx->m, cols = transpose ? ctx->m : ctx->n;
  double* in     = transpose ? ctx->tmp_m : ctx->tmp_n;
  double* outv   = transpose ? ctx->tmp_n : ctx->tmp_m;
  HIP_TRY(hipMemcpyAsync(in, x, (size_t)cols * sizeof(double), hipMemcpyHostToDevice, s));
  launch_plain(ctx, transpose, in, outv);
  LAUNCH_CHECK();
  HIP_TRY(hipMemcpyAsync(y, outv, (size_t)rows * sizeof(double), hipMemcpyDeviceToHost, s));
  HIP_TRY(hipStreamSynchronize(s));
  return 0;
}

int pdlpdev_time_kernel(pdlpdev_ctx* ctx, int kernel_id, int reps, double* avg_ms)
{
  HIP_TRY(hipSetDevice(ctx->device));
  hipStream_t s = ctx->stream;
  if (reps < 1) reps = 1;
  TRY(fetch_ctl(ctx, nullptr));
  loop_state_touched(ctx);
  pdlpdev_ctl saved = *ctx->ctl_h;
  pdlpdev_ctl forced = saved;
  forced.pending_avg  = ctx->halpern ? 0 : 1;
  forced.target_steps = saved.steps_taken + (ctx->halpern ? 2 : 1);
  forced.error        = 0;
  const pdlpdev_halpern saved_hal = ctx->halpern ? *ctx->hal_h : pdlpdev_halpern{};
  double* const keep_n = ctx->halpern ? ctx->avgx : ctx->sumx;
  double* const keep_m = ctx->halpern ? ctx->avgy : ctx->sumy;
  double *sx = nullptr, *sy = nullptr;
  HIP_TRY(hipMalloc((void**)&sx, std::max<size_t>(ctx->n, 1) * sizeof(double)));
  HIP_TRY(hipMalloc((void**)&sy, std::max<size_t>(ctx->m, 1) * sizeof(double)));
  HIP_TRY(hipMemcpyAsync(sx, keep_n, (size_t)ctx->n * sizeof(double), hipMemcpyDeviceToDevice, s));
  HIP_TRY(hipMemcpyAsync(sy, keep_m, (size_t)ctx->m * sizeof(double), hipMemcpyDeviceToDevice, s));
  HIP_TRY(hipMemcpyAsync(ctx->ctl, &forced, sizeof(forced), hipMemcpyHostToDevice, s));
  HIP_TRY(hipStreamSynchronize(s));
  for (hipEvent_t& e : ctx->prof_ev) HIP_TRY(hipEventCreate(&e));
  auto one = [&]() {
    switch (kernel_id) {
      case PDLPDEV_K_PRIMAL:
        launch_k(ctx, k_primal, grid_for(ctx->n), kBlock, 0, ctx->n, ctx->ctl, ctx->x[0], ctx->x[1], ctx->aty[0], ctx->aty[1], ctx->c, ctx->lb, ctx->ub, ctx->xbar, ctx->sumx, (const p2pdev::Push*)nullptr, ctx->ubd);
        break;
      case PDLPDEV_K_SPMV_A_DUAL: launch_a_dual(ctx); break;
      case PDLPDEV_K_SPMV_AT_STEP: launch_at_step(ctx); break;
      case PDLPDEV_K_STEP_DECISION: launch_decision(ctx); break;
      case PDLPDEV_K_SPMV_A_PLAIN:
        launch_plain(ctx, 0, ctx->xbar, ctx->tmp_m);
        break;
      case PDLPDEV_K_SPMV_AT_PLAIN:
        launch_plain(ctx, 1, ctx->y[saved.cur], ctx->tmp_n);
        break;
      default: return fail(-1, "pdlpdev_time_kernel: unknown kernel %d", kernel_id);
    }
    return 0;
  };
  const bool loop_kernel = kernel_id == PDLPDEV_K_PRIMAL || kernel_id == PDLPDEV_K_SPMV_A_DUAL ||
                           kernel_id == PDLPDEV_K_SPMV_AT_STEP || kernel_id == PDLPDEV_K_STEP_DECISION;
  auto attempt = [&](bool timed) -> int {
    const int order[4] = {PDLPDEV_K_PRIMAL, PDLPDEV_K_SPMV_A_DUAL, PDLPDEV_K_SPMV_AT_STEP, PDLPDEV_K_STEP_DECISION};
    const int wanted   = kernel_id;
    const int slot = loop_kernel ? wanted : (wanted == PDLPDEV_K_SPMV_A_PLAIN ? PDLPDEV_K_SPMV_A_DUAL : PDLPDEV_K_SPMV_AT_STEP);
    int rc = 0;
    for (int id : order) {
      const bool mine = id == slot;
      kernel_id       = mine ? wanted : id;
      ctx->prof_armed = mine && timed;
      if (ctx->prof_armed) ctx->prof_used = 0;
      rc              = one();
      ctx->prof_armed = false;
      if (rc != 0) break;
      if (id == PDLPDEV_K_STEP_DECISION)
        HIP_TRY(hipMemcpyAsync(ctx->ctl, &forced, sizeof(forced), hipMemcpyHostToDevice, s));
    }
    kernel_id = wanted;
    return rc;
  };
  TRY(attempt(false));
  float ms = 0.f;
  for (int i = 0; i < reps; ++i) {
    TRY(attempt(true));
    HIP_TRY(hipStreamSynchronize(s));
    for (int q = 0; q < ctx->prof_used; ++q) {
      float one_ms = 0.f;
      HIP_TRY(hipEventElapsedTime(&one_ms, ctx->prof_ev[2 * q], ctx->prof_ev[2 * q + 1]));
      ms += one_ms;
    }
  }
  if (avg_ms) *avg_ms = (double)ms / reps;
  HIP_TRY(hipMemcpyAsync(keep_n, sx, (size_t)ctx->n * sizeof(double), hipMemcpyDeviceToDevice, s));
  HIP_TRY(hipMemcpyAsync(keep_m, sy, (size_t)ctx->m * sizeof(double), hipMemcpyDeviceToDevice, s));
  HIP_TRY(hipMemcpyAsync(ctx->ctl, &saved, sizeof(saved), hipMemcpyHostToDevice, s));
  if (ctx->halpern) HIP_TRY(hipMemcpyAsync(ctx->hal, &saved_hal, sizeof(saved_hal), hipMemcpyHostToDevice, s));
  HIP_TRY(hipStreamSynchronize(s));
  for (hipEvent_t& e : ctx->prof_ev) (void)hipEventDestroy(e), e = nullptr;
  (void)hipFree(sx), (void)hipFree(sy);
  return 0;
}

int pdlpdev_synchronize(pdlpdev_ctx* ctx)
{
  HIP_TRY(hipSetDevice(ctx->device));
  HIP_TRY(hipStreamSynchronize(ctx->stream));
  return 0;
}
int64_t pdlpdev_device_bytes(pdlpdev_ctx* ctx) { return ctx->bytes; }
int pdlpdev_shard_dataflow(pdlpdev_ctx* ctx) { return !ctx->comm ? 0 : ctx->owner ? 3 : ctx->rsag ? 2 : 1; }
int pdlpdev_shard_transport(pdlpdev_ctx* ctx) { return ctx->p2p.on ? 1 : 0; }
int pdlpdev_shard_wire_bytes(pdlpdev_ctx* ctx, int64_t out[3])
{
  out[0] = ctx->halo.on ? 1 : 0, out[1] = ctx->halo.on ? ctx->halo.bytes : ctx->halo.bytes_allgather, out[2] = ctx->halo.bytes_allgather;
  return 0;
}
int pdlpdev_dense_info(pdlpdev_ctx* ctx, int64_t out[3])
{
  out[0] = ctx->dense.on ? 1 : 0, out[1] = ctx->dense.nseg, out[2] = ctx->dense.nent;
  return 0;
}
int pdlpdev_layout_info(pdlpdev_ctx* ctx, int32_t out[8])
{
  ctx->A.info(out), ctx->At.info(out + 3);
  out[6] = ctx->A.pan.on && ctx->A.pan.v.seg, out[7] = ctx->At.pan.on && ctx->At.pan.v.seg;
  if (ctx->small_resident) out[0] = out[3] = 2;
  return 0;
}
// ... 79 lines not shown
```

### cuopt_amd/csrc/pdlp_kernels.hpp

```cpp
#pragma once
#include <hip/hip_runtime.h>
#include <stdint.h>


#include "cuopt_amd/pdlp_device.h"

namespace pdlp {

typedef double vec4d __attribute__((ext_vector_type(4)));
typedef int vec4i __attribute__((ext_vector_type(4)));

constexpr int kBlock    = 256;
constexpr int kNnzTile  = 2048;
constexpr int kNnzBlock = kNnzTile - 4;
constexpr int kLongRow  = 128;
constexpr int kMaxRowsPerBlock = 1024;

template <int XOR_MASK>
__device__ __forceinline__ double swizzle_xor(double v)
{
  static_assert(XOR_MASK >= 1 && XOR_MASK <= 16, "ds_swizzle works inside 32 lanes");
  constexpr int pattern = (XOR_MASK << 10) | 0x1F;
  int lo = __double2loint(v), hi = __double2hiint(v);
  lo = __builtin_amdgcn_ds_swizzle(lo, pattern);
// ... 61 lines not shown
__device__ __forceinline__ double read_lane(double v, int lane)
{
  const int lo = __builtin_amdgcn_readlane(__double2loint(v), lane);
  const int hi = __builtin_amdgcn_readlane(__double2hiint(v), lane);
  return __hiloint2double(hi, lo);
}
__device__ __forceinline__ double wave_sum_dpp(double v)
{
  v = row16_sum(v);
  return ((read_lane(v, 0) + read_lane(v, 16)) + read_lane(v, 32)) + read_lane(v, 48);
}
template <int NQ, int WAVES>
__device__ __forceinline__ void block_sum_fast(double (&v)[NQ], double* scratch )
{
  static_assert(NQ <= 4 && WAVES <= 16, "one DPP row per quantity");
  const int lane = threadIdx.x & 63, wave = threadIdx.x >> 6;
#pragma unroll
  for (int q = 0; q < NQ; ++q) {
    const double w = wave_sum_dpp(v[q]);
    if (lane == 0) scratch[q * 16 + wave] = w;
  }
  __syncthreads();
  const int q = lane >> 4, i = lane & 15;
  double part = (q < NQ && i < WAVES) ? scratch[q * 16 + i] : 0.0;
  part        = row16_sum(part);
#pragma unroll
  for (int k = 0; k < NQ; ++k) v[k] = read_lane(part, 16 * k);
}

__device__ __forceinline__ double dense_plus(const double* __restrict__ add, int r, double v) { return add ? v + add[r] : v; }

__device__ __forceinline__ bool loop_active(const pdlpdev_ctl* ctl)
{
  return ctl->error == 0 && ctl->steps_taken < ctl->target_steps;
}
__device__ __forceinline__ bool period_reached(const pdlpdev_ctl* ctl) { return ctl->steps_taken >= ctl->target_steps; }
constexpr int kPeriodGuard = 0x100;
__device__ __forceinline__ bool period_guard_skips(const pdlpdev_ctl* ctl, int& arg)
{
  const bool guarded = (arg & kPeriodGuard) != 0;
  arg &= ~kPeriodGuard;
  return guarded && !period_reached(ctl);
}

__device__ __forceinline__ int xcd_remap(int b, int nb)
{
  const int per = (nb + 7) >> 3;
  const int v   = (b & 7) * per + (b >> 3);
  return v;
}



constexpr int kPanelThreads = 512;
constexpr int kPanelChunk   = 4096;
constexpr int kPanelMaxRows = 3584;
constexpr int kPanelWaves   = kPanelThreads / 64;

struct PanelView {
  int W, S;
  int any_long;
  const int32_t* __restrict__ row0;
  const int32_t* __restrict__ tile_ptr;
  const uint16_t* __restrict__ rowptr;
  const int64_t* __restrict__ rp_base;
  const int32_t* __restrict__ col;
  const double* __restrict__ val;
  const double* __restrict__ dense_add = nullptr;
  int seg = 0, slab_w = 0;
  int NP = 0;
  const int32_t* __restrict__ own_row = nullptr;
  const int32_t* __restrict__ own_ptr = nullptr;
  const int32_t* __restrict__ csr_off = nullptr;
  const int32_t* __restrict__ csr_idx = nullptr;
  const double* __restrict__ csr_val  = nullptr;
  const int32_t* __restrict__ dn_own_seg   = nullptr;
  const int32_t* __restrict__ dn_pan_ptr   = nullptr;
  const int32_t* __restrict__ dn_pan_seg   = nullptr;
  const int32_t* __restrict__ dn_seg_row   = nullptr;
  const int32_t* __restrict__ dn_seg_c0    = nullptr;
  const int32_t* __restrict__ dn_seg_len   = nullptr;
  const int32_t* __restrict__ dn_seg_ptr   = nullptr;
  const double* __restrict__ dn_val        = nullptr;
};
constexpr int kPanelOwnRow = 4096;
constexpr int kPanelDenseSegs = 32;
constexpr long long kPanelNotMine = 0x7FF8C0DEC0DEC0DELL;

constexpr int kPanelPer     = kPanelChunk / kPanelThreads;
constexpr int kPanelRowsPer = (kPanelMaxRows + kPanelThreads - 1) / kPanelThreads;
constexpr int kSegColBits = 20;
constexpr unsigned kSegColMask = (1u << kSegColBits) - 1u;

constexpr int kJagMaxGroup = 256;
constexpr int kJagBatchRows = 16384;
#ifndef CUOPT_AMD_JAG_U
#define CUOPT_AMD_JAG_U 8
#endif
constexpr int kJagU        = CUOPT_AMD_JAG_U;
constexpr int jag_window(int waves) { return waves == 16 ? 16384 : 8192; }
constexpr size_t jag_lds_bytes(int waves) { return sizeof(double) * (size_t)(jag_window(waves) + waves * kJagMaxGroup); }
constexpr long long kJagNotMine = 0x7FF8C0DEC0DEC0DELL;

struct JagView {
  int rows, waves, ngroups, nblk, nlong;
  const int32_t* __restrict__ row0;
  const int32_t* __restrict__ tile_e;
  const int32_t* __restrict__ tile_sr;
  const uint32_t* __restrict__ sr;
  const uint16_t* __restrict__ slot;
  const double* __restrict__ val;
  const int32_t* __restrict__ win;
  const int32_t* __restrict__ set_ptr;
  const int32_t* __restrict__ set_col;
  const int32_t* __restrict__ lr_ptr;
  const int32_t* __restrict__ lr_row;
  const int32_t* __restrict__ off;
  const int32_t* __restrict__ idx;
  const double* __restrict__ csr_val;
  const double* __restrict__ dense_add = nullptr;
};


constexpr int kPbThreads = 512;
constexpr int kPbCap     = 9088;
constexpr int kPbMaxRows = 1024;
constexpr int kPbKU      = 16;
constexpr size_t kPbLdsBytes = sizeof(double) * (size_t)(kPbCap + kPbMaxRows + 128);
typedef double pb_vec2d __attribute__((ext_vector_type(2)));
constexpr int kPbwRows     = 8192;
constexpr int kPbwStep     = 1024;
constexpr int kPbwThreads  = 1024;
constexpr int kPbwMaxLevel = 6;
constexpr int kPbwAhead    = 4;
constexpr int kPbwMaxSteps = 4096;
constexpr size_t kPbwLdsBytes = sizeof(double) * (size_t)(kPbwRows + 256) + kPbwMaxSteps;

struct PbView {
  int rows, cols, S, B, gshift, panel_shift, nwg;
  const double* __restrict__ val;
  const uint16_t* __restrict__ lidx;
  const int32_t* __restrict__ piece_dst;
  const int32_t* __restrict__ wg_e0;
  const int32_t* __restrict__ wg_panel;
  const int32_t* __restrict__ bin_row0;
  const int32_t* __restrict__ bin_e0;
  const uint32_t* __restrict__ sr;
  const int32_t* __restrict__ bin_grp;
  const int32_t* __restrict__ grp_pos;
  const uint16_t* __restrict__ pos;
  double* __restrict__ prod;
  const double* __restrict__ dense_add = nullptr;
  int wide = 0;
  const uint16_t* __restrict__ rib     = nullptr;
  const uint8_t* __restrict__ step_lv  = nullptr;
  int nser = 0;
  const int32_t* __restrict__ ser_ptr  = nullptr;
  const int32_t* __restrict__ ser_row  = nullptr;
  const int32_t* __restrict__ ser_eptr = nullptr;
  const int32_t* __restrict__ ser_slot = nullptr;
};


__device__ __forceinline__ double dmin(double a, double b) { return a < b ? a : b; }
__device__ __forceinline__ double dmax(double a, double b) { return a > b ? a : b; }
__device__ __forceinline__ bool dfinite(double v) { return fabs(v) <= 1.7976931348623157e308; }
__device__ __forceinline__ double combine_bounds(double lower, double upper)
// ... 124 lines not shown
```

### cuopt_amd/csrc/spmv_panel.hpp

```cpp
#pragma once
#include <type_traits>

#include "pdlp_kernels.hpp"

namespace pdlp {

struct PanelChunk {
  int s, c0, c1, t0;
  bool valid;
};
template <int R>
__device__ __forceinline__ void panel_load(const PanelView& P, double (&va)[kPanelPer], int (&ja)[kPanelPer], int c0, int c1)
{
#pragma unroll
  for (int u = 0; u < R; ++u) {
    int k = c0 + threadIdx.x + u * kPanelThreads;
    if (u == R - 1) k = k < c1 ? k : c1 - 1;
    va[u] = __builtin_nontemporal_load(P.val + k);
    ja[u] = __builtin_nontemporal_load(P.col + k);
  }
}
template <int R>
__device__ __forceinline__ void panel_products(const double* __restrict__ vec, double* prod, const double (&va)[kPanelPer],
                                               const int (&ja)[kPanelPer], int len)
{
  double x[R];
#pragma unroll
  for (int u = 0; u < R; ++u) x[u] = vec[ja[u]];
#pragma unroll
  for (int u = 0; u < R; ++u) {
    const int i = threadIdx.x + u * kPanelThreads;
    if (u < R - 1 || i < len) prod[i] = va[u] * x[u];
  }
}
#define PANEL_DISPATCH(rounds, CALL) \
  switch (rounds) {                   \
    case 1: CALL(1); break;           \
    case 2: CALL(2); break;           \
    case 3: CALL(3); break;           \
    case 4: CALL(4); break;           \
    case 5: CALL(5); break;           \
    case 6: CALL(6); break;           \
    case 7: CALL(7); break;           \
    default: CALL(8); break;          \
  }

template <class Epi>
__device__ __forceinline__ void panel_own_row(const PanelView& P, const double* __restrict__ vec, Epi& epi, double* __restrict__ partials,
                                              int w, int NP, double* scratch )
{
  const int r  = P.own_row[w - NP];
  const int k0 = P.csr_off[r], k1 = P.csr_off[r + 1];
  double part[1] = {0.0};
  constexpr int kLongU = 16;
  for (int k = k0 + (int)threadIdx.x; k < k1; k += kLongU * kPanelThreads) {
    double a[kLongU];
    int j[kLongU];
#pragma unroll
    for (int u = 0; u < kLongU; ++u) {
      a[u] = 0.0, j[u] = 0;
      if (k + u * kPanelThreads < k1) {
        a[u] = __builtin_nontemporal_load(P.csr_val + k + u * kPanelThreads);
        j[u] = __builtin_nontemporal_load(P.csr_idx + k + u * kPanelThreads);
      }
    }
    double xv[kLongU];
#pragma unroll
    for (int u = 0; u < kLongU; ++u) xv[u] = k + u * kPanelThreads < k1 ? vec[j[u]] : 0.0;
#pragma unroll
    for (int u = 0; u < kLongU; ++u) part[0] = part[0] + a[u] * xv[u];
  }
  if (P.dn_own_seg) {
    for (int sg = P.dn_own_seg[w - NP]; sg < P.dn_own_seg[w - NP + 1]; ++sg) {
      const int len = P.dn_seg_len[sg];
      const double* __restrict__ a = P.dn_val + P.dn_seg_ptr[sg];
      const double* __restrict__ x = vec + P.dn_seg_c0[sg];
      constexpr int kSegU = 8;
      for (int k = (int)threadIdx.x; k < len; k += kSegU * kPanelThreads) {
        double av[kSegU], xv[kSegU];
#pragma unroll
        for (int u = 0; u < kSegU; ++u) {
          const int i = k + u * kPanelThreads;
          av[u] = i < len ? __builtin_nontemporal_load(a + i) : 0.0;
          xv[u] = i < len ? x[i] : 0.0;
        }
#pragma unroll
        for (int u = 0; u < kSegU; ++u) part[0] = part[0] + av[u] * xv[u];
      }
    }
  }
  block_reduce<SumOp, 1, kPanelWaves>(part, scratch);
  double acc[Epi::NQ > 0 ? Epi::NQ : 1];
#pragma unroll
  for (int q = 0; q < (Epi::NQ > 0 ? Epi::NQ : 1); ++q) acc[q] = Epi::Op::identity();
  if (threadIdx.x == 0) {
    epi.row(r, dense_plus(P.dense_add, r, part[0]), acc);
    if constexpr (Epi::NQ > 0) {
#pragma unroll
      for (int q = 0; q < Epi::NQ; ++q) partials[(size_t)q * P.W + w] = acc[q];
    }
  }
}
struct PanelDenseSegs {
  int n;
  int c0[kPanelDenseSegs], len[kPanelDenseSegs], ptr[kPanelDenseSegs];
  double y[kPanelDenseSegs];
};
__device__ __forceinline__ void panel_dense_prepare(const PanelView& P, int w, const double* __restrict__ vec, PanelDenseSegs* D)
{
  if (!P.dn_pan_ptr) return;
  const int q0 = P.dn_pan_ptr[w], n = P.dn_pan_ptr[w + 1] - q0;
  if (threadIdx.x == 0) D->n = n;
  if ((int)threadIdx.x < n) {
    const int sg = P.dn_pan_seg[q0 + threadIdx.x];
    D->c0[threadIdx.x] = P.dn_seg_c0[sg], D->len[threadIdx.x] = P.dn_seg_len[sg], D->ptr[threadIdx.x] = P.dn_seg_ptr[sg];
// ... 69 lines not shown
template <class Epi>
__device__ __forceinline__ void panel_epilogue_early(const PanelView& P, Epi& epi, double* __restrict__ partials, const double* psum, double* red,
                                                     int w, int r0, int nr, const PanelDenseSegs* D,
                                                     const typename Epi::Ops (&pre)[kPanelEpiDepth], const double* psum2 = nullptr)
{
  double acc[Epi::NQ > 0 ? Epi::NQ : 1];
#pragma unroll
  for (int q = 0; q < (Epi::NQ > 0 ? Epi::NQ : 1); ++q) acc[q] = Epi::Op::identity();
  __builtin_amdgcn_s_waitcnt(0x0F70);
#pragma unroll
  for (int q = 0; q < kPanelEpiDepth; ++q) {
    const int r = threadIdx.x + q * kPanelThreads;
    if (r < nr && __double_as_longlong(psum[r]) != kPanelNotMine) {
      double v = psum2 ? psum[r] + psum2[r] : psum[r];
      if (P.dn_pan_ptr) v = v + panel_dense_col(P, D, r0 + r);
      epi.apply(r0 + r, dense_plus(P.dense_add, r0 + r, v), pre[q], acc);
    }
  }
  panel_epilogue_rows(P, epi, acc, psum, threadIdx.x + kPanelEpiDepth * kPanelThreads, r0, nr, D, psum2);
  panel_epilogue_partials<Epi>(P, partials, acc, red, w);
}

__device__ __forceinline__ void panel_row_sums(const PanelView& P, const unsigned (&ext)[kPanelRowsPer], const double* prod, double* psum,
                                               int nr, int lo, int hi)
{
  if (!P.any_long) {
#pragma unroll
    for (int q = 0; q < kPanelRowsPer; ++q) {
      const int r = threadIdx.x + q * kPanelThreads;
      if (r < nr) {
        int a = (int)(ext[q] & 0xFFFFu), b = (int)(ext[q] >> 16);
        a = a > lo ? a : lo;
        b = b < hi ? b : hi;
        if (a < b) {
          double sum = psum[r];
          for (int k = a; k < b; ++k) sum = sum + prod[k - lo];
          psum[r] = sum;
        }
      }
    }
    return;
  }
  bool any_long = false;
#pragma unroll
  for (int q = 0; q < kPanelRowsPer; ++q) {
    const int r = threadIdx.x + q * kPanelThreads;
    if (r < nr) {
      int a = (int)(ext[q] & 0xFFFFu), b = (int)(ext[q] >> 16);
      a = a > lo ? a : lo;
      b = b < hi ? b : hi;
      if (b - a > kLongRow) {
        any_long = true;
      } else if (a < b) {
        double sum = psum[r];
        for (int k = a; k < b; ++k) sum = sum + prod[k - lo];
        psum[r] = sum;
      }
    }
  }
  if (__ballot(any_long)) {
#pragma unroll
    for (int q = 0; q < kPanelRowsPer; ++q) {
      const int r = threadIdx.x + q * kPanelThreads;
      int a = 0, b = 0;
      if (r < nr) {
        a = (int)(ext[q] & 0xFFFFu), b = (int)(ext[q] >> 16);
        a = a > lo ? a : lo;
        b = b < hi ? b : hi;
      }
      unsigned long long todo = __ballot(b - a > kLongRow);
      while (todo) {
        const int l  = __builtin_ctzll(todo);
        todo &= todo - 1;
        const int la = __builtin_amdgcn_readlane(a, l), lb = __builtin_amdgcn_readlane(b, l);
        double part  = 0.0;
        for (int k = la + (int)(threadIdx.x & 63); k < lb; k += 64) part = part + prod[k - lo];
        part = wave_reduce<SumOp>(part);
        if ((int)(threadIdx.x & 63) == l) psum[r] = psum[r] + part;
      }
    }
  }
}

template <class Epi>
__device__ __forceinline__ void panel_spmv_block(const PanelView& P, const double* __restrict__ vec,
                                                 Epi& epi, double* __restrict__ partials)
{
  static_assert(kPanelPer == 8, "PANEL_DISPATCH enumerates 1..8 rounds");
  __shared__ double prod[kPanelChunk];
  __shared__ double psum[kPanelMaxRows];
  __shared__ double red[kPanelWaves * (Epi::NQ > 0 ? Epi::NQ : 1)];
  __shared__ int tile_s[17];
  __shared__ long long base_s[16];
  const int w  = blockIdx.x;
  const int NP = P.NP ? P.NP : P.W;
  if (w >= NP) {
    panel_own_row(P, vec, epi, partials, w, NP, prod);
    return;
  }
  __shared__ PanelDenseSegs dseg;
  const int r0 = P.row0[w], nr = P.row0[w + 1] - r0;
  panel_dense_prepare(P, w, vec, &dseg);
  if (threadIdx.x <= P.S) tile_s[threadIdx.x] = P.tile_ptr[w * P.S + threadIdx.x];
  if (threadIdx.x < P.S) base_s[threadIdx.x] = P.rp_base[w * P.S + threadIdx.x];
  for (int r = threadIdx.x; r < nr; r += kPanelThreads) psum[r] = 0.0;
  __syncthreads();
  if (P.own_ptr)
    for (int q = P.own_ptr[w] + (int)threadIdx.x; q < P.own_ptr[w + 1]; q += kPanelThreads) psum[P.own_row[q] - r0] = __longlong_as_double(kPanelNotMine);
  auto advance = [&](PanelChunk c) -> PanelChunk {
    if (c.valid && c.c1 < tile_s[c.s + 1]) {
      c.c0 = c.c1;
      c.c1 = c.c0 + kPanelChunk < tile_s[c.s + 1] ? c.c0 + kPanelChunk : tile_s[c.s + 1];
      return c;
    }
    int s = c.s + 1;
    while (s < P.S && tile_s[s + 1] == tile_s[s]) ++s;
    c.valid = s < P.S;
    c.s     = s;
    if (c.valid) {
      c.t0 = c.c0 = tile_s[s];
      c.c1 = c.c0 + kPanelChunk < tile_s[s + 1] ? c.c0 + kPanelChunk : tile_s[s + 1];
    }
    return c;
  };
  double va[kPanelPer];
  int ja[kPanelPer];
  unsigned ext_next[kPanelRowsPer], ext[kPanelRowsPer];
#define PANEL_ROUNDS(c) (((c).c1 - (c).c0 + kPanelThreads - 1) / kPanelThreads)
#define PANEL_CALL_LOAD(R) panel_load<R>(P, va, ja, nxt.c0, nxt.c1)
#define PANEL_CALL_PRODUCTS(R) panel_products<R>(vec, prod, va, ja, cur.c1 - cur.c0)
#define PANEL_REQUEST(c)                                                         \
  if ((c).valid) {                                                               \
    PANEL_DISPATCH(PANEL_ROUNDS(c), PANEL_CALL_LOAD)                             \
    const uint16_t* __restrict__ rp_ = P.rowptr + base_s[(c).s];                 \
    _Pragma("unroll") for (int q = 0; q < kPanelRowsPer; ++q) {                  \
      int r_      = threadIdx.x + q * kPanelThreads;                             \
      r_          = r_ < nr ? r_ : 0;                                            \
      ext_next[q] = (unsigned)rp_[r_] | ((unsigned)rp_[r_ + 1] << 16);           \
    }                                                                            \
  }
  PanelChunk none{-1, 0, 0, 0, false};
  PanelChunk nxt = advance(none);
  PANEL_REQUEST(nxt)
  PanelChunk cur = nxt;
  constexpr bool kEarly = PanelEarlyOps<Epi>::on;
  [[maybe_unused]] typename PanelEarlyOps<Epi>::type pre[kPanelEpiDepth];
  [[maybe_unused]] int lo_last = 0, hi_last = 0;
  while (cur.valid) {
    __syncthreads();
    PANEL_DISPATCH(PANEL_ROUNDS(cur), PANEL_CALL_PRODUCTS)
#pragma unroll
    for (int q = 0; q < kPanelRowsPer; ++q) ext[q] = ext_next[q];
    const int lo = cur.c0 - cur.t0, hi = cur.c1 - cur.t0;
    nxt = advance(cur);
    if constexpr (kEarly)
      if (!nxt.valid) {
        lo_last = lo, hi_last = hi;
        break;
      }
    PANEL_REQUEST(nxt)
    __syncthreads();
    panel_row_sums(P, ext, prod, psum, nr, lo, hi);
    cur = nxt;
  }
#undef PANEL_REQUEST
#undef PANEL_CALL_PRODUCTS
#undef PANEL_CALL_LOAD
#undef PANEL_ROUNDS
  if constexpr (kEarly) {
    panel_epilogue_request(epi, pre, r0, nr);
    if (cur.valid) {
      __syncthreads();
      panel_row_sums(P, ext, prod, psum, nr, lo_last, hi_last);
    }
    __syncthreads();
    panel_epilogue_early(P, epi, partials, psum, red, w, r0, nr, &dseg, pre);
  } else {
    __syncthreads();
    panel_epilogue(P, epi, partials, psum, red, w, r0, nr, &dseg);
  }
}
template <int CTRL, int ROW_MASK>
__device__ __forceinline__ double seg_dpp(double v)
{
  int lo = __double2loint(v), hi = __double2hiint(v);
  lo = __builtin_amdgcn_update_dpp(0, lo, CTRL, ROW_MASK, 0xf, false);
  hi = __builtin_amdgcn_update_dpp(0, hi, CTRL, ROW_MASK, 0xf, false);
  return __hiloint2double(hi, lo);
}
__device__ __forceinline__ double seg_scan(double S, int lane, int seg0)
{
  double u;
  u = seg_dpp<0x111, 0xf>(S); if ((lane & 15) >= 1 && lane - 1 >= seg0) S = S + u;
  u = seg_dpp<0x112, 0xf>(S); if ((lane & 15) >= 2 && lane - 2 >= seg0) S = S + u;
  u = seg_dpp<0x114, 0xf>(S); if ((lane & 15) >= 4 && lane - 4 >= seg0) S = S + u;
  u = seg_dpp<0x118, 0xf>(S); if ((lane & 15) >= 8 && lane - 8 >= seg0) S = S + u;
  u = seg_dpp<0x142, 0xa>(S); if ((lane & 16) && (lane | 15) - 16 >= seg0) S = S + u;
  u = seg_dpp<0x143, 0xc>(S); if (lane >= 32 && 31 >= seg0) S = S + u;
  return S;
}
__device__ __forceinline__ void seg_emit(double* strip, int row, double v)
{
  __hip_atomic_fetch_add(strip + row, v, __ATOMIC_RELAXED, __HIP_MEMORY_SCOPE_WORKGROUP);
}
struct SegRecord {
  double lsum, rsum;
  int lkey, rkey;
};
template <int R>
__device__ __forceinline__ void seg_load(const PanelView& P, double (&va)[kPanelPer], int (&pk)[kPanelPer], int c0, int c1)
{
#pragma unroll
  for (int u = 0; u < R; ++u) {
    int k = c0 + threadIdx.x + u * kPanelThreads;
    if (u == R - 1) k = k < c1 ? k : c1 - 1;
    va[u] = __builtin_nontemporal_load(P.val + k);
    pk[u] = __builtin_nontemporal_load(P.col + k);
  }
}
template <int R>
__device__ __forceinline__ void seg_rounds(const double* __restrict__ vec, int slab_base, const double (&va)[kPanelPer], const int (&pk)[kPanelPer], int len,
                                           double* psum, SegRecord* rec , int lane)
{
  double x[R];
#pragma unroll
  for (int u = 0; u < R; ++u) x[u] = vec[slab_base + (int)((unsigned)pk[u] & kSegColMask)];
#pragma unroll
  for (int u = 0; u < R; ++u) {
    const int i   = threadIdx.x + u * kPanelThreads;
    const int key = (int)((unsigned)pk[u] >> kSegColBits);
    const double v = (u < R - 1 || i < len) ? va[u] * x[u] : 0.0;
    const int prev = __builtin_amdgcn_update_dpp(-1, key, 0x138, 0xf, 0xf, false);
    const unsigned long long starts = __ballot(key != prev);
    const unsigned long long below  = starts & ((2ull << lane) - 1ull);
    const int seg0                  = 63 - __builtin_clzll(below);
    const double S                  = seg_scan(v, lane, seg0);
    const bool ends                 = lane == 63 || ((starts >> (lane + 1)) & 1ull);
    if (ends) {
      if (seg0 == 0) {
        rec[u].lsum = S, rec[u].lkey = key;
        if (lane == 63) rec[u].rkey = -1;
      } else if (lane == 63) {
        rec[u].rsum = S, rec[u].rkey = key;
      } else {
        seg_emit(psum, key, S);
      }
    }
  }
// ... 44 lines not shown
  const int w  = blockIdx.x;
  const int NP = P.NP ? P.NP : P.W;
  if (w >= NP) {
    panel_own_row(P, vec, epi, partials, w, NP, psum);
    return;
  }
  __shared__ PanelDenseSegs dseg;
  const int r0 = P.row0[w], nr = P.row0[w + 1] - r0;
  panel_dense_prepare(P, w, vec, &dseg);
  if (threadIdx.x <= P.S) tile_s[threadIdx.x] = P.tile_ptr[w * P.S + threadIdx.x];
  for (int r = threadIdx.x; r < nr; r += kPanelThreads) psum[r] = 0.0, psum2[r] = 0.0;
  __syncthreads();
  if (P.own_ptr)
    for (int q = P.own_ptr[w] + (int)threadIdx.x; q < P.own_ptr[w + 1]; q += kPanelThreads) psum[P.own_row[q] - r0] = __longlong_as_double(kPanelNotMine);
  auto advance = [&](PanelChunk c) -> PanelChunk {
    if (c.valid && c.c1 < tile_s[c.s + 1]) {
      c.c0 = c.c1;
      c.c1 = c.c0 + kPanelChunk < tile_s[c.s + 1] ? c.c0 + kPanelChunk : tile_s[c.s + 1];
      return c;
    }
    int s = c.s + 1;
    while (s < P.S && tile_s[s + 1] == tile_s[s]) ++s;
    c.valid = s < P.S;
    c.s     = s;
    if (c.valid) {
      c.t0 = c.c0 = tile_s[s];
      c.c1 = c.c0 + kPanelChunk < tile_s[s + 1] ? c.c0 + kPanelChunk : tile_s[s + 1];
    }
    return c;
  };
  const int lane = threadIdx.x & 63;
  const int wave = __builtin_amdgcn_readfirstlane(threadIdx.x >> 6);
  double va[kPanelPer];
  int pk[kPanelPer];
#define SEG_ROUNDS(c) (((c).c1 - (c).c0 + kPanelThreads - 1) / kPanelThreads)
#define SEG_CALL_LOAD(R) seg_load<R>(P, va, pk, nxt.c0, nxt.c1)
#define SEG_CALL_ROUNDS(R) seg_rounds<R>(vec, cur.s * P.slab_w, va, pk, cur.c1 - cur.c0, psum, &rec[parity][wave * kPanelPer], lane)
  PanelChunk none{-1, 0, 0, 0, false};
  PanelChunk nxt = advance(none);
  if (nxt.valid) { PANEL_DISPATCH(SEG_ROUNDS(nxt), SEG_CALL_LOAD) }
  PanelChunk cur = nxt;
  int parity = 0;
  constexpr bool kEarly = PanelEarlyOps<Epi>::on;
  [[maybe_unused]] typename PanelEarlyOps<Epi>::type pre[kPanelEpiDepth];
  [[maybe_unused]] int R_last = 0;
  while (cur.valid) {
    const int R = SEG_ROUNDS(cur);
    PANEL_DISPATCH(R, SEG_CALL_ROUNDS)
    nxt = advance(cur);
    if constexpr (kEarly)
      if (!nxt.valid) {
        R_last = R;
        break;
      }
    if (nxt.valid) { PANEL_DISPATCH(SEG_ROUNDS(nxt), SEG_CALL_LOAD) }
    __syncthreads();
    if (wave == 0) panel_seg_join(rec[parity], psum2, R, lane);
    parity ^= 1;
    cur = nxt;
  }
#undef SEG_CALL_ROUNDS
#undef SEG_CALL_LOAD
#undef SEG_ROUNDS
  if constexpr (kEarly) {
    panel_epilogue_request(epi, pre, r0, nr);
    if (cur.valid) {
      __syncthreads();
      if (wave == 0) panel_seg_join(rec[parity], psum2, R_last, lane);
    }
    __syncthreads();
    panel_epilogue_early(P, epi, partials, psum, red, w, r0, nr, &dseg, pre, psum2);
  } else {
    __syncthreads();
    panel_epilogue(P, epi, partials, psum, red, w, r0, nr, &dseg, psum2);
  }
}
#undef PANEL_DISPATCH
template <bool SEG, class Epi>
__device__ __forceinline__ void panel_block(const PanelView& P, const double* __restrict__ vec, Epi& epi, double* __restrict__ partials)
{
  if constexpr (SEG) panel_seg_block(P, vec, epi, partials);
  else panel_spmv_block(P, vec, epi, partials);
}

}
```

### include/cuopt_amd/pdlp_device.h

```cpp
#ifndef CUOPT_AMD_PDLP_DEVICE_H
#define CUOPT_AMD_PDLP_DEVICE_H

#include <stdint.h>

#ifdef __cplusplus
extern "C" {
#endif

typedef struct pdlpdev_ctx pdlpdev_ctx;

typedef struct pdlpdev_ctl {
  double step_size;
  double primal_weight;
  double tau;
  double sigma;
  double sum_weights;
  double last_interaction, last_movement, last_dx2, last_dy2;
  int32_t k;
  int32_t cur;
  int32_t pending_avg;
  int32_t steps_taken;
  int32_t attempts;
  int32_t target_steps;
  int32_t error;
  int32_t its_since_restart;
} pdlpdev_ctl;

typedef struct pdlpdev_halpern {
  double r;
  double r_first;
  double r2;
  double r2_min;
  int32_t k;
  int32_t reserved;
} pdlpdev_halpern;

typedef struct pdlpdev_step_params {
  double reduction_exponent;
  double growth_exponent;
  double primal_distance_smoothing;
  double dual_distance_smoothing;
} pdlpdev_step_params;

enum {
  PDLPDEV_EV_CX = 0,
  PDLPDEV_EV_DUAL_SUM,
  PDLPDEV_EV_PRES2,
  PDLPDEV_EV_DRES2,
  PDLPDEV_EV_X2,
  PDLPDEV_EV_Y2,
  PDLPDEV_EV_LINF_PRES_REL,
  PDLPDEV_EV_LINF_DRES_REL,
  PDLPDEV_EV_COUNT
};

enum {
  PDLPDEV_CURRENT = 0,
  PDLPDEV_AVERAGE = 1,
  PDLPDEV_LAST_RESTART = 2,
  PDLPDEV_BEST = 3
};

enum {
  PDLPDEV_BUF_X = 0,
  PDLPDEV_BUF_Y,
  PDLPDEV_BUF_X_OTHER,
  PDLPDEV_BUF_Y_OTHER,
  PDLPDEV_BUF_ATY,
  PDLPDEV_BUF_ATY_OTHER,
  PDLPDEV_BUF_XBAR,
  PDLPDEV_BUF_SUM_X,
  PDLPDEV_BUF_SUM_Y,
  PDLPDEV_BUF_AVG_X,
  PDLPDEV_BUF_AVG_Y,
  PDLPDEV_BUF_DROW,
  PDLPDEV_BUF_DCOL,
  PDLPDEV_BUF_A_VALUES,
  PDLPDEV_BUF_AT_VALUES,
  PDLPDEV_BUF_C,
  PDLPDEV_BUF_LB, PDLPDEV_BUF_UB,
  PDLPDEV_BUF_LO, PDLPDEV_BUF_HI,
  PDLPDEV_BUF_RC_CURRENT,
  PDLPDEV_BUF_RC_AVERAGE,
  PDLPDEV_BUF_LAST_RESTART_X, PDLPDEV_BUF_LAST_RESTART_Y,
  PDLPDEV_BUF_ATY_U_CURRENT,
  PDLPDEV_BUF_ATY_U_AVERAGE,
  PDLPDEV_BUF_LAST_RESTART_ATY,
  PDLPDEV_BUF_AX_U_CURRENT,
  PDLPDEV_BUF_AX_U_AVERAGE,
  PDLPDEV_BUF_COUNT
};

enum {
  PDLPDEV_K_PRIMAL = 0,
  PDLPDEV_K_SPMV_A_DUAL,
  PDLPDEV_K_SPMV_AT_STEP,
  PDLPDEV_K_STEP_DECISION,
  PDLPDEV_K_SPMV_A_PLAIN,
  PDLPDEV_K_SPMV_AT_PLAIN,
  PDLPDEV_K_ITERATION,
  PDLPDEV_K_COUNT
};

const char* pdlpdev_last_error(void);
int pdlpdev_device_count(void);
int pdlpdev_device_info(int dev, char* name, int len, int* compute_units, int64_t* hbm_bytes);

int pdlpdev_create(pdlpdev_ctx** out, int device, int32_t m, int32_t n, const int32_t* a_offsets,
                   const int32_t* a_indices, const double* a_values, const int32_t* at_offsets,
                   const int32_t* at_indices, const double* at_values, const double* c,
                   const double* lo, const double* hi, const double* lb, const double* ub);
void pdlpdev_create_hint(int sharded);
void pdlpdev_create_no_resident(int no_resident);
void pdlpdev_create_batch_lanes(int lanes);
void pdlpdev_create_share_stream(pdlpdev_ctx* donor);
int pdlpdev_resident_size(int32_t m, int32_t n, int64_t nnz);
int pdlpdev_resident_tier(int32_t m, int32_t n, int64_t nnz);
int pdlpdev_create_overlapped(pdlpdev_ctx** out, int device, int32_t m, int32_t n, const int32_t* a_offsets,
                              const int32_t* a_indices, const double* a_values, const int32_t* at_offsets,
                              const int32_t* at_indices, const double* at_values,
                              void (*transpose_ready)(void*), void* user, const double* c, const double* lo,
                              const double* hi, const double* lb, const double* ub);
void pdlpdev_destroy(pdlpdev_ctx* ctx);

typedef struct pdlpdev_analysis pdlpdev_analysis;
int pdlpdev_analyze(pdlpdev_analysis** out, int device, int32_t m, int32_t n, const int32_t* a_offsets, const int32_t* a_indices,
                    const double* a_values, int flags);
int pdlpdev_analyze_with_vectors(pdlpdev_analysis** out, int device, int32_t m, int32_t n, const int32_t* a_offsets, const int32_t* a_indices,
                                 const double* a_values, int flags, const double* c, const double* lo, const double* hi, const double* lb,
                                 const double* ub);
int pdlpdev_analysis_info(pdlpdev_analysis* an, int32_t out[10]);
int pdlpdev_analysis_maps(pdlpdev_analysis* an, int32_t* row_new2old, int32_t* col_new2old);
int pdlpdev_analysis_vectors_in_order(pdlpdev_analysis* an);
void pdlpdev_analysis_release_workspace(pdlpdev_analysis* an);
int pdlpdev_analysis_download(pdlpdev_analysis* an, int which, int32_t* offsets, int32_t* indices, double* values);
int pdlpdev_create_from_analysis(pdlpdev_ctx** out, pdlpdev_analysis* an, const double* c, const double* lo, const double* hi,
                                 const double* lb, const double* ub);
void pdlpdev_analysis_destroy(pdlpdev_analysis* an);
int pdlpdev_debug_sort_pairs(int device, int64_t n, const uint32_t* keys, const uint32_t* vals, int bits, uint32_t* keys_out,
                             uint32_t* vals_out);
int pdlpdev_debug_scan(int device, int64_t n, const int32_t* in, int32_t* out);
int pdlpdev_debug_ipc_export(int device, int count, uint8_t handle[64], void** base);
int pdlpdev_debug_ipc_store(int device, const uint8_t handle[64], int count, double seed);
int pdlpdev_debug_ipc_wait(int device, void* base, int count, double seed);
int pdlpdev_debug_layout_checksums(pdlpdev_ctx* ctx, uint64_t out[16]);
int pdlpdev_debug_pb_wide_host(int32_t rows, int32_t cols, const int32_t* off, const int32_t* idx, const double* val, const double* x, double* out,
                               int64_t info[5]);
int pdlpdev_synthetic_lp(int device, int32_t m, int32_t n, int32_t k, uint64_t seed, int32_t* offsets, int32_t* indices, double* values,
                         double* c, double* lo, double* hi, double* x_star, double* y_star);

int pdlpdev_comm_unique_id(uint8_t id[128]);
int pdlpdev_comm_init(pdlpdev_ctx* ctx, int rank, int world, const uint8_t id[128]);

int pdlpdev_softcomm_create(int world, uint8_t id[128]);
int pdlpdev_comm_abort(const uint8_t id[128]);

int pdlpdev_scaling_compute(pdlpdev_ctx* ctx, int do_ruiz, int ruiz_iterations,
                            int do_pock_chambolle, double alpha);
int pdlpdev_scale_problem(pdlpdev_ctx* ctx);
int pdlpdev_init_norms(pdlpdev_ctx* ctx, double out[3]);
int pdlpdev_agree_max(pdlpdev_ctx* ctx, double* value);
int pdlpdev_weight_norms(pdlpdev_ctx* ctx, int unscaled, double out[2]);
int pdlpdev_reset(pdlpdev_ctx* ctx, const double* lb, const double* ub, const double* lo, const double* hi);
int pdlpdev_problem_norms(pdlpdev_ctx* ctx, double* norm_c, double* norm_b);
int pdlpdev_set_step_params(pdlpdev_ctx* ctx, const pdlpdev_step_params* p);
int pdlpdev_set_step(pdlpdev_ctx* ctx, double step_size, double primal_weight);
int pdlpdev_set_k(pdlpdev_ctx* ctx, int32_t k);
int pdlpdev_set_initial(pdlpdev_ctx* ctx, const double* x, const double* y);
int pdlpdev_project_primal(pdlpdev_ctx* ctx);
int pdlpdev_initial_solution_stats(pdlpdev_ctx* ctx, double out[5], const double* x0_unscaled, const double* y0_unscaled);

int pdlpdev_compute_aty(pdlpdev_ctx* ctx);
// ... 91 lines not shown
```

Measured before the change: 6240 iterations/s.

## Skip gathers of zero xbar entries in panel SpMV using a ballot bitmap

The primal kernel now writes a per-column nonzero bitmap of xbar via wavefront ballots and counts nonzeros per block. The step-decision kernel sums those counts and sets a hysteresis flag in the control struct when xbar is sparse enough. When the flag is set, the A·xbar panel SpMV stages the bitmap slice in shared memory and skips gathering x entries that are zero, saving memory traffic. The cost is extra bitmap writes, a count reduction, more shared memory and a branchier product loop, and it only pays off when many xbar entries are zero.

Measured after the change: 6588 iterations/s, median of 6. 1.06x the previous value.

```diff
diff --git a/cuopt_amd/capi.py b/cuopt_amd/capi.py
--- a/cuopt_amd/capi.py
+++ b/cuopt_amd/capi.py
@@ -42,7 +42,7 @@
                 ("last_movement", c_double), ("last_dx2", c_double), ("last_dy2", c_double),
                 ("k", c_int), ("cur", c_int), ("pending_avg", c_int), ("steps_taken", c_int),
                 ("attempts", c_int), ("target_steps", c_int), ("error", c_int),
-                ("its_since_restart", c_int)]
+                ("its_since_restart", c_int), ("zskip", c_int), ("zs_nonzeros", c_int)]
 
 
 class StepParams(C.Structure):
@@ -350,7 +350,7 @@
     ["X", "Y", "X_OTHER", "Y_OTHER", "ATY", "ATY_OTHER", "XBAR", "SUM_X", "SUM_Y", "AVG_X", "AVG_Y",
      "DROW", "DCOL", "A_VALUES", "AT_VALUES", "C", "LB", "UB", "LO", "HI", "RC_CURRENT", "RC_AVERAGE",
      "LAST_RESTART_X", "LAST_RESTART_Y", "ATY_U_CURRENT", "ATY_U_AVERAGE", "LAST_RESTART_ATY",
-     "AX_U_CURRENT", "AX_U_AVERAGE"])}
+     "AX_U_CURRENT", "AX_U_AVERAGE", "PART_A", "PART_AT", "XBAR_MASK", "ZS_LAUNCHES"])}
 KERNEL = {n: i for i, n in enumerate(
     ["PRIMAL", "SPMV_A_DUAL", "SPMV_AT_STEP", "STEP_DECISION", "SPMV_A_PLAIN", "SPMV_AT_PLAIN"])}
 EV = {n: i for i, n in enumerate(
diff --git a/cuopt_amd/csrc/kernels_batch.hip b/cuopt_amd/csrc/kernels_batch.hip
--- a/cuopt_amd/csrc/kernels_batch.hip
+++ b/cuopt_amd/csrc/kernels_batch.hip
@@ -529,6 +529,7 @@
   c->parent = nullptr;
   c->scal_h = nullptr, c->ctl_h = nullptr;
   c->halpern = false, c->lraty = nullptr, c->hal = nullptr, c->hal_h = nullptr;
+  c->xmask = nullptr, c->zcount = nullptr, c->zs_mode = 0;
   c->clones_alive = 0, c->batches_alive = 0, c->rows_private = false;
   c->bytes = 0, c->slab = nullptr, c->slab_cap = c->slab_used = 0, c->arena = nullptr, c->arena_used = 0, c->first_chunk = nullptr;
   c->bestx = c->besty = c->bestrc = nullptr;
diff --git a/cuopt_amd/csrc/kernels_panel.hip b/cuopt_amd/csrc/kernels_panel.hip
--- a/cuopt_amd/csrc/kernels_panel.hip
+++ b/cuopt_amd/csrc/kernels_panel.hip
@@ -14,7 +14,10 @@
 {
   if (!loop_active(ctl)) return;
   DualEpilogue e = DualEpilogue::make(ctl, y0, y1, lo, hi, sumy, ycopy, push);
-  panel_block<SEG>(P, xbar, e, part);
+  const bool masked = !SEG && P.zmask != nullptr && (P.zforce != 0 || ctl->zskip != 0);
+  if (masked && blockIdx.x == 0 && threadIdx.x == 0)
+    __hip_atomic_fetch_add(const_cast<unsigned long long*>(P.zmask) + 2 * ((size_t)(P.zcols + 127) / 128), 1ull, __ATOMIC_RELAXED, __HIP_MEMORY_SCOPE_AGENT);
+  panel_block_zs<SEG>(P, xbar, e, part, masked);
   if (push) p2pdev::count_exchange(push);
 }
 
diff --git a/cuopt_amd/csrc/pdlp_create.hip b/cuopt_amd/csrc/pdlp_create.hip
--- a/cuopt_amd/csrc/pdlp_create.hip
+++ b/cuopt_amd/csrc/pdlp_create.hip
@@ -552,6 +552,13 @@
     TRY(pick_layout(ctx, &ctx->At, ctx->tmp_m, ctx->tmp_n));
     lap("layout autotune");
   }
+  if (one_gpu && !ctx->small_resident && ctx->A.layout() == pdlpdev_ctx::MatrixSide::kPanel && !ctx->A.pan.v.seg && cuopt_amd::tune_int("zero_skip", 1) != 0) {
+    const size_t words = 2 * (((size_t)n + 127) / 128);
+    ctx->zs_mode = cuopt_amd::tune_int("zero_skip", 1) == 2 ? 2 : 1;
+    TRY(dev_alloc(ctx, &ctx->zcount, (size_t)grid_for(n)));
+    TRY(dev_alloc(ctx, &ctx->xmask, words + 2));
+    HIP_TRY(hipMemsetAsync(ctx->xmask, 0, (words + 2) * sizeof(unsigned long long), ctx->stream));
+  }
   HIP_TRY(hipStreamSynchronize(ctx->stream));
   scratch_free(ctx);
   return 0;
diff --git a/cuopt_amd/csrc/pdlp_ctx.hpp b/cuopt_amd/csrc/pdlp_ctx.hpp
--- a/cuopt_amd/csrc/pdlp_ctx.hpp
+++ b/cuopt_amd/csrc/pdlp_ctx.hpp
@@ -382,6 +382,9 @@
   bool scaled = false;
   double *x[2] = {nullptr, nullptr}, *y[2] = {nullptr, nullptr}, *aty[2] = {nullptr, nullptr};
   double *xbar = nullptr, *sumx = nullptr, *sumy = nullptr, *avgx = nullptr, *avgy = nullptr;
+  unsigned long long* xmask = nullptr;
+  int* zcount = nullptr;
+  int zs_mode = 0;
   double *lrx = nullptr, *lry = nullptr, *rc[2] = {nullptr, nullptr};
   double *tmp_n = nullptr, *tmp_m = nullptr;
   double *ax_u[3] = {nullptr, nullptr, nullptr}, *aty_u[3] = {nullptr, nullptr, nullptr};
diff --git a/cuopt_amd/csrc/pdlp_device.hip b/cuopt_amd/csrc/pdlp_device.hip
--- a/cuopt_amd/csrc/pdlp_device.hip
+++ b/cuopt_amd/csrc/pdlp_device.hip
@@ -107,12 +107,15 @@
   finalize_rows(part, nb, nq, op_mask, out, red);
 }
 
-__global__ void __launch_bounds__(kBlock)
-k_primal(int n, const pdlpdev_ctl* __restrict__ ctl, double* __restrict__ x0, double* __restrict__ x1,
+template <bool ZS>
+__device__ __forceinline__ void
+primal_body(int n, const pdlpdev_ctl* __restrict__ ctl, double* __restrict__ x0, double* __restrict__ x1,
          const double* __restrict__ aty0, const double* __restrict__ aty1,
          const double* __restrict__ c, const double* __restrict__ lb, const double* __restrict__ ub,
-         double* __restrict__ xbar, double* __restrict__ sumx, const p2pdev::Push* __restrict__ push, pdlpdev_ctx::UniformBounds ubd)
-{
+         double* __restrict__ xbar, double* __restrict__ sumx, const p2pdev::Push* __restrict__ push, pdlpdev_ctx::UniformBounds ubd,
+         unsigned long long* __restrict__ xmask, int* __restrict__ zcount)
+{
+  [[maybe_unused]] int nz = 0;
   if (!loop_active(ctl)) return;
   const int cur       = ctl->cur;
   const double tau    = ctl->tau;
@@ -129,12 +132,45 @@
     xn[j]                 = next;
     const double xb       = next - xj + next;
     xbar[j]               = xb;
+    if constexpr (ZS) {
+      const unsigned long long bits = __ballot(xb != 0.0);
+      if ((threadIdx.x & 63) == 0) xmask[j >> 6] = bits;
+      nz += __popcll(bits);
+    }
     if (push)
       for (int q = 0; q < push->world; ++q)
         if (push->wants(q, j)) p2pdev::put(push->slot(q) + j, xb);
     if (pend) sumx[j] = sumx[j] + weight * xj;
   }
+  if constexpr (ZS) {
+    __shared__ int wave_nz[kBlock / 64];
+    if ((threadIdx.x & 63) == 0) wave_nz[threadIdx.x >> 6] = nz;
+    __syncthreads();
+    if (threadIdx.x == 0) {
+      int sum = 0;
+#pragma unroll
+      for (int w = 0; w < kBlock / 64; ++w) sum += wave_nz[w];
+      zcount[blockIdx.x] = sum;
+    }
+  }
   if (push) p2pdev::count_exchange(push);
+}
+__global__ void __launch_bounds__(kBlock)
+k_primal(int n, const pdlpdev_ctl* __restrict__ ctl, double* __restrict__ x0, double* __restrict__ x1,
+         const double* __restrict__ aty0, const double* __restrict__ aty1,
+         const double* __restrict__ c, const double* __restrict__ lb, const double* __restrict__ ub,
+         double* __restrict__ xbar, double* __restrict__ sumx, const p2pdev::Push* __restrict__ push, pdlpdev_ctx::UniformBounds ubd)
+{
+  primal_body<false>(n, ctl, x0, x1, aty0, aty1, c, lb, ub, xbar, sumx, push, ubd, nullptr, nullptr);
+}
+__global__ void __launch_bounds__(kBlock)
+k_primal_zs(int n, const pdlpdev_ctl* __restrict__ ctl, double* __restrict__ x0, double* __restrict__ x1,
+            const double* __restrict__ aty0, const double* __restrict__ aty1,
+            const double* __restrict__ c, const double* __restrict__ lb, const double* __restrict__ ub,
+            double* __restrict__ xbar, double* __restrict__ sumx, pdlpdev_ctx::UniformBounds ubd,
+            unsigned long long* __restrict__ xmask, int* __restrict__ zcount)
+{
+  primal_body<true>(n, ctl, x0, x1, aty0, aty1, c, lb, ub, xbar, sumx, nullptr, ubd, xmask, zcount);
 }
 
 
@@ -169,11 +205,13 @@
 
 constexpr int kDecisionThreads = 1024;
 static_assert(kDecisionThreads == kHalpernDecisionThreads, "k_halpern_decision runs halpern_decision_workgroup");
+template <bool ZS = false>
 __device__ __forceinline__ void step_decision_workgroup(pdlpdev_ctl* __restrict__ ctl, const double* __restrict__ part_dy, int nb_dy,
                                                         const double* __restrict__ part_t, int nb_t, const double* __restrict__ dy2_reduced,
-                                                        const pdlpdev_step_params& sp)
-{
-  __shared__ double red[3 * 16];
+                                                        const pdlpdev_step_params& sp, const int* __restrict__ zcount = nullptr, int nb_z = 0,
+                                                        int zn = 0, int zmode = 0)
+{
+  __shared__ double red[(ZS ? 4 : 3) * 16];
   __shared__ double pw[2];
   pdlpdev_ctl lc = *ctl;
   if (!(lc.error == 0 && lc.steps_taken < lc.target_steps)) return;
@@ -182,7 +220,7 @@
     const double knext = (double)(lc.k + 1) + 1.0;
     pw[t - (kDecisionThreads - 2)] = pow(knext, t == kDecisionThreads - 2 ? -sp.reduction_exponent : -sp.growth_exponent);
   }
-  double acc[3] = {0.0, 0.0, 0.0};
+  double acc[ZS ? 4 : 3] = {0.0, 0.0, 0.0};
   if (dy2_reduced == nullptr) {
 #pragma unroll 4
     for (int i = t; i < nb_dy; i += kDecisionThreads) acc[0] += part_dy[i];
@@ -192,10 +230,23 @@
     acc[1] += part_t[i];
     acc[2] += part_t[nb_t + i];
   }
-  block_sum_fast<3, kDecisionThreads / 64>(acc, red);
+  if constexpr (ZS) {
+    acc[3] = 0.0;
+#pragma unroll 2
+    for (int i = t; i < nb_z; i += kDecisionThreads) acc[3] += (double)zcount[i];
+  }
+  block_sum_fast<ZS ? 4 : 3, kDecisionThreads / 64>(acc, red);
   if (t != 0) return;
   apply_step_decision(&lc, dy2_reduced ? dy2_reduced[0] : acc[0], acc[1], acc[2], sp, pw);
-  *ctl = lc;
+  if constexpr (ZS) {
+    const long long nonzeros = (long long)acc[3];
+    lc.zs_nonzeros           = (int32_t)nonzeros;
+    if (zmode == 2 || nonzeros * 4 <= 3ll * zn) lc.zskip = 1;
+    else if (nonzeros * 100 >= 87ll * zn) lc.zskip = 0;
+    *ctl = lc;
+  } else {
+    __builtin_memcpy(ctl, &lc, offsetof(pdlpdev_ctl, zskip));
+  }
 }
 __global__ void __launch_bounds__(kDecisionThreads)
 k_step_decision(pdlpdev_ctl* __restrict__ ctl, const double* __restrict__ part_dy, int nb_dy,
@@ -203,6 +254,12 @@
                 pdlpdev_step_params sp)
 {
   step_decision_workgroup(ctl, part_dy, nb_dy, part_t, nb_t, dy2_reduced, sp);
+}
+__global__ void __launch_bounds__(kDecisionThreads)
+k_step_decision_zs(pdlpdev_ctl* __restrict__ ctl, const double* __restrict__ part_dy, int nb_dy,
+                   const double* __restrict__ part_t, int nb_t, pdlpdev_step_params sp, const int* __restrict__ zcount, int nb_z, int zn, int zmode)
+{
+  step_decision_workgroup<true>(ctl, part_dy, nb_dy, part_t, nb_t, nullptr, sp, zcount, nb_z, zn, zmode);
 }
 __global__ void __launch_bounds__(kDecisionThreads)
 k_step_decision_batch(const pdlpdev_decision_args* __restrict__ args)
@@ -792,8 +849,23 @@
 
 
 static inline HalpernArgs halpern_args(const pdlpdev_ctx* ctx) { return HalpernArgs{ctx->hal, ctx->avgx, ctx->avgy, ctx->lrx, ctx->lry, ctx->lraty}; }
+static unsigned long long* attempt_xmask(const pdlpdev_ctx* ctx)
+{
+  const pdlpdev_ctx::Panels& pn = ctx->A.pan;
+  if (!ctx->xmask || ctx->comm || ctx->owner || ctx->rsag || ctx->halpern) return nullptr;
+  if (ctx->A.layout() != pdlpdev_ctx::MatrixSide::kPanel || pn.v.seg) return nullptr;
+  return ctx->xmask;
+}
+static void launch_primal(pdlpdev_ctx* ctx)
+{
+  const int n = ctx->n;
+  if (unsigned long long* xmask = attempt_xmask(ctx))
+    return launch_k(ctx, k_primal_zs, grid_for(n), kBlock, 0, n, ctx->ctl, ctx->x[0], ctx->x[1], ctx->aty[0], ctx->aty[1], ctx->c, ctx->lb, ctx->ub, ctx->xbar, ctx->sumx, ctx->ubd, xmask, ctx->zcount);
+  launch_k(ctx, k_primal, grid_for(n), kBlock, 0, n, ctx->ctl, ctx->x[0], ctx->x[1], ctx->aty[0], ctx->aty[1], ctx->c, ctx->lb, ctx->ub, ctx->xbar, ctx->sumx, (const p2pdev::Push*)nullptr, ctx->ubd);
+}
 static void launch_a_dual(pdlpdev_ctx* ctx, double* ycopy = nullptr, const p2pdev::Push* push = nullptr)
 {
+  ctx->A.pan.v.zmask = attempt_xmask(ctx), ctx->A.pan.v.zcols = ctx->n, ctx->A.pan.v.zforce = ctx->zs_mode == 2;
   const Gathered g = Gathered::fixed(ctx->xbar, true);
   const auto pre  = std::make_tuple(ctx->ctl);
   const auto vecs = std::make_tuple(ctx->xbar);
@@ -822,6 +894,9 @@
 static void launch_decision(pdlpdev_ctx* ctx)
 {
   if (ctx->halpern) return launch_k(ctx, k_halpern_decision, 1, kDecisionThreads, 0, ctx->ctl, ctx->hal, ctx->A.part, ctx->A.partials(), ctx->At.part, ctx->At.partials());
+  if (attempt_xmask(ctx))
+    return launch_k(ctx, k_step_decision_zs, 1, kDecisionThreads, 0, ctx->ctl, ctx->A.part, ctx->A.partials(), ctx->At.part, ctx->At.partials(), ctx->sp, ctx->zcount,
+                    grid_for(ctx->n), ctx->n, ctx->zs_mode);
   launch_k(ctx, k_step_decision, 1, kDecisionThreads, 0, ctx->ctl, ctx->A.part, ctx->A.partials(), ctx->At.part, ctx->At.partials(), nullptr, ctx->sp);
 }
 
@@ -907,7 +982,7 @@
     LAUNCH_CHECK();
     return 0;
   }
-  launch_k(ctx, k_primal, grid_for(n), kBlock, 0, n, ctx->ctl, ctx->x[0], ctx->x[1], ctx->aty[0], ctx->aty[1], ctx->c, ctx->lb, ctx->ub, ctx->xbar, ctx->sumx, (const p2pdev::Push*)nullptr, ctx->ubd);
+  launch_primal(ctx);
   launch_a_dual(ctx);
   if (!ctx->comm) {
     launch_at_step(ctx);
@@ -1281,6 +1356,16 @@
       break;
     case PDLPDEV_BUF_AX_U_CURRENT: src = ctx->ax_u[PDLPDEV_CURRENT], count = m; break;
     case PDLPDEV_BUF_AX_U_AVERAGE: src = ctx->ax_u[PDLPDEV_AVERAGE], count = m; break;
+    case PDLPDEV_BUF_PART_A: src = ctx->A.part, count = ctx->A.partials(); break;
+    case PDLPDEV_BUF_PART_AT: src = ctx->At.part, count = 2 * (int64_t)ctx->At.partials(); break;
+    case PDLPDEV_BUF_ZS_LAUNCHES:
+      if (!ctx->xmask) { fail(-1, "buffer %d: this context has no bitmap of xbar (CUOPT_AMD_TUNE=zero_skip=0, or A is not in the row-sum panels)", id); return -1; }
+      src = reinterpret_cast<double*>(ctx->xmask + 2 * (((size_t)n + 127) / 128)), count = 1;
+      break;
+    case PDLPDEV_BUF_XBAR_MASK:
+      if (!ctx->xmask) { fail(-1, "buffer %d: this context has no bitmap of xbar (CUOPT_AMD_TUNE=zero_skip=0, or A is not in the row-sum panels)", id); return -1; }
+      src = reinterpret_cast<double*>(ctx->xmask), count = (n + 63) / 64;
+      break;
     default: fail(-1, "unknown buffer %d", id); return -1;
   }
   *ptr = src;
@@ -1307,6 +1392,10 @@
   if (count < 0) return count;
   if (id == PDLPDEV_BUF_A_VALUES || id == PDLPDEV_BUF_AT_VALUES) {
     fail(-1, "matrix values cannot be overwritten");
+    return -1;
+  }
+  if (id == PDLPDEV_BUF_XBAR_MASK || id == PDLPDEV_BUF_ZS_LAUNCHES || id == PDLPDEV_BUF_PART_A || id == PDLPDEV_BUF_PART_AT) {
+    fail(-1, "the bitmap of xbar and the reduction partials are written by the attempt's kernels alone");
     return -1;
   }
   count = std::min(count, elements);
@@ -1455,7 +1544,7 @@
   auto one = [&]() {
     switch (kernel_id) {
       case PDLPDEV_K_PRIMAL:
-        launch_k(ctx, k_primal, grid_for(ctx->n), kBlock, 0, ctx->n, ctx->ctl, ctx->x[0], ctx->x[1], ctx->aty[0], ctx->aty[1], ctx->c, ctx->lb, ctx->ub, ctx->xbar, ctx->sumx, (const p2pdev::Push*)nullptr, ctx->ubd);
+        launch_primal(ctx);
         break;
       case PDLPDEV_K_SPMV_A_DUAL: launch_a_dual(ctx); break;
       case PDLPDEV_K_SPMV_AT_STEP: launch_at_step(ctx); break;
diff --git a/cuopt_amd/csrc/pdlp_kernels.hpp b/cuopt_amd/csrc/pdlp_kernels.hpp
--- a/cuopt_amd/csrc/pdlp_kernels.hpp
+++ b/cuopt_amd/csrc/pdlp_kernels.hpp
@@ -167,7 +167,10 @@
   const int32_t* __restrict__ dn_seg_len   = nullptr;
   const int32_t* __restrict__ dn_seg_ptr   = nullptr;
   const double* __restrict__ dn_val        = nullptr;
-};
+  const unsigned long long* __restrict__ zmask = nullptr;
+  int zcols = 0, zforce = 0;
+};
+constexpr int kZsQuads        = 1152;
 constexpr int kPanelOwnRow = 4096;
 constexpr int kPanelDenseSegs = 32;
 constexpr long long kPanelNotMine = 0x7FF8C0DEC0DEC0DELL;
diff --git a/cuopt_amd/csrc/spmv_panel.hpp b/cuopt_amd/csrc/spmv_panel.hpp
--- a/cuopt_amd/csrc/spmv_panel.hpp
+++ b/cuopt_amd/csrc/spmv_panel.hpp
@@ -31,6 +31,53 @@
   for (int u = 0; u < R; ++u) {
     const int i = threadIdx.x + u * kPanelThreads;
     if (u < R - 1 || i < len) prod[i] = va[u] * x[u];
+  }
+}
+template <int R>
+__device__ __forceinline__ void panel_products_zs(const double* __restrict__ vec, double* prod, const double (&va)[kPanelPer],
+                                                  const int (&ja)[kPanelPer], int len, const unsigned* zbits, int zbase)
+{
+  unsigned w[R];
+#pragma unroll
+  for (int u = 0; u < R; ++u) {
+    const int wi = (ja[u] >> 5) - zbase;
+    w[u]         = wi < kZsQuads * 4 ? zbits[wi] : ~0u;
+  }
+  double x[R];
+#pragma unroll
+  for (int u = 0; u < R; ++u) {
+    x[u] = 0.0;
+    if ((w[u] >> (ja[u] & 31)) & 1u) x[u] = vec[ja[u]];
+  }
+#pragma unroll
+  for (int u = 0; u < R; ++u) {
+    const int i = threadIdx.x + u * kPanelThreads;
+    if (u < R - 1 || i < len) prod[i] = va[u] * x[u];
+  }
+}
+constexpr int kZsPer = (kZsQuads + kPanelThreads - 1) / kPanelThreads;
+__device__ __forceinline__ int panel_zs_first_quad(const PanelView& P, int s) { return (int)(((long long)s * P.slab_w) >> 7); }
+__device__ __forceinline__ void panel_zs_load(const PanelView& P, int s, uint4 (&st)[kZsPer])
+{
+  const long long c1 = (long long)(s + 1) * P.slab_w;
+  const int last     = (int)(c1 < P.zcols ? c1 : P.zcols) - 1;
+  const int q0       = panel_zs_first_quad(P, s);
+  int nq             = (last >> 7) - q0 + 1;
+  nq                 = nq < kZsQuads ? nq : kZsQuads;
+  const uint4* __restrict__ src = reinterpret_cast<const uint4*>(P.zmask) + q0;
+#pragma unroll
+  for (int k = 0; k < kZsPer; ++k) {
+    const int q = threadIdx.x + k * kPanelThreads;
+    st[k]       = uint4{0u, 0u, 0u, 0u};
+    if (q < nq) st[k] = src[q];
+  }
+}
+__device__ __forceinline__ void panel_zs_store(uint4* zq, const uint4 (&st)[kZsPer])
+{
+#pragma unroll
+  for (int k = 0; k < kZsPer; ++k) {
+    const int q = threadIdx.x + k * kPanelThreads;
+    if (q < kZsQuads) zq[q] = st[k];
   }
 }
 #define PANEL_DISPATCH(rounds, CALL) \
@@ -266,11 +313,17 @@
   }
 }
 
-template <class Epi>
+template <class Epi, bool ZS = false>
 __device__ __forceinline__ void panel_spmv_block(const PanelView& P, const double* __restrict__ vec,
-                                                 Epi& epi, double* __restrict__ partials)
+                                                 Epi& epi, double* __restrict__ partials, const unsigned long long* zmask = nullptr)
 {
   static_assert(kPanelPer == 8, "PANEL_DISPATCH enumerates 1..8 rounds");
+  [[maybe_unused]] uint4* zq = nullptr;
+  if constexpr (ZS) {
+    __shared__ uint4 zq_s[kZsQuads];
+    zq = zq_s;
+  }
+  const bool zon = ZS && zmask != nullptr;
   __shared__ double prod[kPanelChunk];
   __shared__ double psum[kPanelMaxRows];
   __shared__ double red[kPanelWaves * (Epi::NQ > 0 ? Epi::NQ : 1)];
@@ -313,6 +366,7 @@
 #define PANEL_ROUNDS(c) (((c).c1 - (c).c0 + kPanelThreads - 1) / kPanelThreads)
 #define PANEL_CALL_LOAD(R) panel_load<R>(P, va, ja, nxt.c0, nxt.c1)
 #define PANEL_CALL_PRODUCTS(R) panel_products<R>(vec, prod, va, ja, cur.c1 - cur.c0)
+#define PANEL_CALL_PRODUCTS_ZS(R) panel_products_zs<R>(vec, prod, va, ja, cur.c1 - cur.c0, reinterpret_cast<const unsigned*>(zq), panel_zs_first_quad(P, cur.s) << 2)
 #define PANEL_REQUEST(c)                                                         \
   if ((c).valid) {                                                               \
     PANEL_DISPATCH(PANEL_ROUNDS(c), PANEL_CALL_LOAD)                             \
@@ -327,12 +381,18 @@
   PanelChunk nxt = advance(none);
   PANEL_REQUEST(nxt)
   PanelChunk cur = nxt;
+  if (zon && cur.valid) {
+    uint4 st[kZsPer];
+    panel_zs_load(P, cur.s, st);
+    panel_zs_store(zq, st);
+  }
   constexpr bool kEarly = PanelEarlyOps<Epi>::on;
   [[maybe_unused]] typename PanelEarlyOps<Epi>::type pre[kPanelEpiDepth];
   [[maybe_unused]] int lo_last = 0, hi_last = 0;
   while (cur.valid) {
     __syncthreads();
-    PANEL_DISPATCH(PANEL_ROUNDS(cur), PANEL_CALL_PRODUCTS)
+    if (zon) { PANEL_DISPATCH(PANEL_ROUNDS(cur), PANEL_CALL_PRODUCTS_ZS) }
+    else { PANEL_DISPATCH(PANEL_ROUNDS(cur), PANEL_CALL_PRODUCTS) }
 #pragma unroll
     for (int q = 0; q < kPanelRowsPer; ++q) ext[q] = ext_next[q];
     const int lo = cur.c0 - cur.t0, hi = cur.c1 - cur.t0;
@@ -344,10 +404,18 @@
       }
     PANEL_REQUEST(nxt)
     __syncthreads();
-    panel_row_sums(P, ext, prod, psum, nr, lo, hi);
+    if (zon && nxt.valid && nxt.s != cur.s) {
+      uint4 st[kZsPer];
+      panel_zs_load(P, nxt.s, st);
+      panel_row_sums(P, ext, prod, psum, nr, lo, hi);
+      panel_zs_store(zq, st);
+    } else {
+      panel_row_sums(P, ext, prod, psum, nr, lo, hi);
+    }
     cur = nxt;
   }
 #undef PANEL_REQUEST
+#undef PANEL_CALL_PRODUCTS_ZS
 #undef PANEL_CALL_PRODUCTS
 #undef PANEL_CALL_LOAD
 #undef PANEL_ROUNDS
@@ -558,5 +626,11 @@
   if constexpr (SEG) panel_seg_block(P, vec, epi, partials);
   else panel_spmv_block(P, vec, epi, partials);
 }
-
-}
+template <bool SEG, class Epi>
+__device__ __forceinline__ void panel_block_zs(const PanelView& P, const double* __restrict__ vec, Epi& epi, double* __restrict__ partials, bool on)
+{
+  if constexpr (SEG) panel_seg_block(P, vec, epi, partials);
+  else panel_spmv_block<Epi, true>(P, vec, epi, partials, on ? P.zmask : nullptr);
+}
+
+}
diff --git a/include/cuopt_amd/pdlp_device.h b/include/cuopt_amd/pdlp_device.h
--- a/include/cuopt_amd/pdlp_device.h
+++ b/include/cuopt_amd/pdlp_device.h
@@ -24,6 +24,8 @@
   int32_t target_steps;
   int32_t error;
   int32_t its_since_restart;
+  int32_t zskip;
+  int32_t zs_nonzeros;
 } pdlpdev_ctl;
 
 typedef struct pdlpdev_halpern {
@@ -88,6 +90,10 @@
   PDLPDEV_BUF_LAST_RESTART_ATY,
   PDLPDEV_BUF_AX_U_CURRENT,
   PDLPDEV_BUF_AX_U_AVERAGE,
+  PDLPDEV_BUF_PART_A,
+  PDLPDEV_BUF_PART_AT,
+  PDLPDEV_BUF_XBAR_MASK,
+  PDLPDEV_BUF_ZS_LAUNCHES,
   PDLPDEV_BUF_COUNT
 };
 
```
